# lzzcd001/MeshDiffusion

Measured on NVIDIA H100. Metric: denoising sample-steps/sec at res-64 (4x64^3), uncond_gen PC sampler, higher is better.
Workload: dtype bf16x3

## Files before the change

### include/meshdiff_b200.h

```cpp
#ifndef MESHDIFF_B200_H
#define MESHDIFF_B200_H

#ifdef __cplusplus
extern "C" {
#endif

const char* mdb_last_error(void);
int mdb_version(void);

typedef struct mdb_unet mdb_unet;

typedef struct mdb_unet_config {
  int image_size;
  int nf;
  int n_levels;
  int ch_mult[8];
  int num_res_blocks;
  int level0_blocks;
  int n_attn;
  int attn_resolutions[4];
  int num_channels;
  int stem_ksize;
  int use_pos_bias;
  int max_batch;
  int precision;
  int training;
} mdb_unet_config;

int mdb_unet_create(const mdb_unet_config* cfg, mdb_unet** out);
int mdb_unet_create_dry(const mdb_unet_config* cfg, mdb_unet** out);
void mdb_unet_destroy(mdb_unet* net);

int mdb_unet_num_params(mdb_unet* net);
int mdb_unet_param_info(mdb_unet* net, int idx, const char** name, long long* numel, int* ndim, long long* shape8);
int mdb_unet_set_param(mdb_unet* net, const char* name, const float* src, long long numel, int src_is_device,
                       void* stream);
int mdb_unet_set_params(mdb_unet* net, int count, const char* const* names, const float* const* srcs, const long long* numels,
                        void* stream);
int mdb_unet_get_param(mdb_unet* net, const char* name, float* dst, long long numel, int dst_is_device, void* stream);
int mdb_unet_commit(mdb_unet* net, void* stream);
int mdb_unet_forward(mdb_unet* net, const float* x, const float* labels, float* out, int batch, void* stream);
int mdb_unet_info(mdb_unet* net, double* flops_per_sample, long long* arena_bytes, int* n_gemm_launches, int* n_steps);
int mdb_unet_gemm_ops(mdb_unet* net, int i, const char** name, double* flops, double* fill_bytes);
int mdb_unet_gemm_slots(mdb_unet* net, int i, int* a_slots, int* b_slots, int* smem_bytes);
int mdb_unet_gemm_tiles(mdb_unet* net, int i, int* work_items, int* splits, int* ksteps, int* entry_ksteps, int* block_n);
int mdb_unet_profile(mdb_unet* net, const float* x, const float* labels, float* out, int batch, void* stream,
                     char* names_buf, int names_len, float* ms, int max_steps, int* n_steps);

int mdb_unet_set_dropout(mdb_unet* net, float p, unsigned long long seed);
int mdb_unet_backward(mdb_unet* net, const float* dout, float* grads, long long grads_numel, int batch, int accumulate,
                      void* stream);
int mdb_unet_grad_offset(mdb_unet* net, const char* name, long long* offset);
int mdb_unet_backward_input(mdb_unet* net, const float* dout, float* dx, float* grads, long long grads_numel, int batch,
                            int accumulate, void* stream);
int mdb_unet_grad_ready(mdb_unet* net, const char* name, int* n_launches);
int mdb_unet_backward_marked(mdb_unet* net, const float* dout, float* grads, long long grads_numel, int batch,
                             int accumulate, const int* mark_steps, void* const* mark_events, int n_marks, void* stream);
int mdb_unet_debug_stats(mdb_unet* net, long long* host_out, long long capacity, long long* count);
int mdb_unet_train_info(mdb_unet* net, double* bwd_flops_per_sample, int* n_bwd_steps, long long* total_param_numel);
int mdb_unet_profile_backward(mdb_unet* net, const float* dout, float* grads, int batch, void* stream, char* names_buf,
                              int names_len, float* ms, int max_steps, int* n_steps);

int mdb_fingerprint(const void* const* ptrs_dev, const long long* numels_dev, int n, unsigned long long* out_dev,
                    void* stream);

typedef struct mdb_sampler_cond {
  const float* partial;
  long long partial_bstride;
  const float* partial_mask;
  long long mask_bstride;
  int channel;
  float mean_coef, std;
  const float* noise;
} mdb_sampler_cond;

int mdb_sampler_update(const float* eps, float* x, float* x_mean, const float* noise, const float* mask, float beta,
                       float std, long long voxels, int channels, int batch, unsigned long long seed,
                       unsigned long long offset, const mdb_sampler_cond* cond , void* stream);
int mdb_sampler_run(mdb_unet* net, float* x, float* x_mean, const float* mask, const float* labels,
                    const float* betas, const float* stds, int n_steps, int batch, unsigned long long seed,
                    float* eps_buf, float* labels_buf, int step0, const mdb_sampler_cond* cond ,
                    const float* cond_mean_coefs, const float* cond_stds, int cond_until, void* stream);

typedef struct mdb_solver_step {
  float label;
  float sigma, inv_alpha;
  float c_x, c_0, c_1, c_z;
  float cond_coef, cond_std;
} mdb_solver_step;

int mdb_solver_update(const float* eps, float* x, float* x0_hist, const float* mask, const mdb_solver_step* step,
                      long long voxels, int channels, int batch, const float* noise ,
                      unsigned long long seed, unsigned long long offset, const mdb_sampler_cond* cond ,
                      void* stream);
int mdb_solver_run(mdb_unet* net, float* x, float* x0_hist, const float* mask, const mdb_solver_step* steps, int n_steps,
                   int batch, unsigned long long seed, float* eps_buf, float* labels_buf, int step0,
                   const mdb_sampler_cond* cond , int cond_until, void* stream);

typedef struct mdb_repaint_entry {
  int kind;
  float label;
  float sigma, inv_alpha;
  float c_x, c_0, c_1, c_z;
  float known_coef, known_std;
} mdb_repaint_entry;

typedef struct mdb_repaint_known {
  const float* known;
  long long known_bstride;
  const float* mask;
  long long mask_bstride;
  unsigned channels;
  const float* noise;
} mdb_repaint_known;

int mdb_repaint_update(const float* eps, float* x, float* x0_hist, const float* mask, const mdb_repaint_entry* entry,
                       long long voxels, int channels, int batch, const float* noise ,
                       unsigned long long seed, unsigned long long offset, const mdb_repaint_known* known ,
                       void* stream);
int mdb_repaint_run(mdb_unet* net, float* x, float* x0_hist, const float* mask, const mdb_repaint_entry* entries,
                    int n_entries, int batch, unsigned long long seed, float* eps_buf, float* labels_buf, int step0,
                    const mdb_repaint_known* known , void* stream);

int mdb_ddpm_loss(const float* pred, const float* noise, const float* mask, double mask_sum, float* loss_out,
                  float* grad_pred, double* scratch, int batch, int channels, long long voxels, void* stream);
int mdb_ddpm_perturb(const float* x0, const float* noise, const float* mask, const float* sqrt_ac,
                     const float* sqrt_1mac, float* out, int batch, int channels, long long voxels, void* stream);
int mdb_chunk_elems(void);
int mdb_grad_clip_coef(const float* const* grads_dev, const long long* numels_dev, const int* chunks_dev, int n_chunks,
                       float max_norm, float* coef_out, float* total_norm_out, double* scratch, void* stream);
int mdb_adam_ema_step(float* const* params_dev, const float* const* grads_dev, float* const* exp_avg_dev,
                      float* const* exp_avg_sq_dev, float* const* ema_dev, const long long* numels_dev,
                      const int* chunks_dev, int n_chunks, float lr, float beta1, float beta2, float eps,
                      float weight_decay, int step, const float* clip_coef_dev, float ema_decay, void* stream);
int mdb_ema_update(float* const* ema_dev, const float* const* params_dev, const long long* numels_dev,
                   const int* chunks_dev, int n_chunks, float ema_decay, void* stream);

int mdb_allreduce_grads(void* nccl_comm, float* grads, long long numel, int world_size, void* stream);

int mdb_conv3d(const void* x, int batch, int cin, int z, int y_, int x_, const float* w, const float* bias, int cout,
               int ksize, int stride, void* out, const float* rowbias, const void* residual, long long* stats,
               int precision, void* stream);
int mdb_groupnorm_act(const void* x, const long long* stats, const float* gamma, const float* beta, void* y, int batch,
                      long long voxels, int channels, int silu, int precision, void* stream);

int mdb_conv3d_backward(const void* dy, const void* x, const float* w, int batch, int cin, int cout, int z, int y_,
                        int x_, int ksize, int stride, float* dw, void* dx, void* stream);
int mdb_conv3d_backward_prec(const void* dy, const void* x, const float* w, int batch, int cin, int cout, int z, int y_,
                             int x_, int ksize, int stride, float* dw, void* dx, int precision, void* stream);
int mdb_groupnorm_act_backward(const void* x, const long long* stats, const float* gamma, const float* beta,
                               void* da, const void* add, void* dx, float* dgamma, float* dbeta, int batch,
                               long long voxels, int channels, int silu, float dropout_p, unsigned long long seed,
                               void* stream);
int mdb_groupnorm_act_backward_prec(const void* x, const long long* stats, const float* gamma, const float* beta,
                                    void* da, const void* add, void* dx, float* dgamma, float* dbeta, int batch,
                                    long long voxels, int channels, int silu, float dropout_p, unsigned long long seed,
                                    int precision, void* stream);

int mdb_marching_tets_prepare(const int* tets_host, int n_tets, int n_verts, int max_batch, void** handle);
void mdb_marching_tets_destroy(void* handle);
int mdb_marching_tets_info(void* handle, int* n_edges, int* uv_grid_n);
int mdb_marching_tets_uvs(void* handle, float* uvs, void* stream);
int mdb_marching_tets_count(void* handle, const float* sdf, int batch, int* counts_host, void* stream);
int mdb_marching_tets_extract(void* handle, const float* pos, long long pos_batch_stride, const float* sdf, int batch,
                              float* verts, long long* faces, long long* uv_idx, long long* face_to_tet,
                              long long* valid_vert_idx, const long long* vert_off, const long long* face_off,
                              const long long* vv_off, void* stream);
int mdb_marching_tets_vertex_ids(void* handle, int batch, unsigned* out, void* stream);
int mdb_marching_tets_backward(void* handle, const float* pos, long long pos_batch_stride, const float* sdf, int batch,
                               const unsigned* vertex_ids, const float* grad_verts, const long long* vert_off,
                               float* grad_pos, float* grad_sdf, void* stream);

int mdb_mesh_auto_normals(const float* v_pos, const long long* faces, int n_verts, int n_faces, float* v_nrm, float* f_nrm,
                          long long* scratch, void* stream);
int mdb_mesh_compute_tangents(const float* v_pos, const long long* t_pos_idx, const float* v_tex, const long long* t_tex_idx,
                              const float* v_nrm, const long long* t_nrm_idx, int n_nrm, int n_faces, float* v_tng,
                              long long* scratch, void* stream);

int mdb_mesh_sample_points(const float* verts, const long long* faces, const long long* vert_off, const long long* face_off,
                           int n_meshes, int n_points, const float* uniforms, unsigned long long seed, long long first_id,
                           double* cdf, float* points, int* n_written, void* stream);
int mdb_chamfer_matrix(const float* A, int nA, int N, const float* B, int nB, int M, double* out, void* stream);
int mdb_chamfer_pairs(const float* clouds, int n_clouds, int N, const int* pairs, int P, double* cd, double* mean_ab,
                      float* max_ab, void* stream);
int mdb_emd_matrix(const float* A, int nA, const float* B, int nB, int N, float eps, double* out, double* gap, void* stream);
int mdb_lfd_descriptors(const int* face_id, int n_images, int res, const float* ray_cs, const double* dft,
                        unsigned char* desc, int* n_inside, void* stream);
int mdb_lfd_matrix(const unsigned char* A, int nA, const unsigned char* B, int nB, const signed char* perms, int* out,
                   void* stream);

int mdb_pflow_drift_div(const float* x, const float* e, const float* h, const float* g, const float* mask, float beta, float std,
                        float* drift, double* div, int batch, int channels, long long voxels, void* stream);

int mdb_raster_depth(const float* verts, const long long* faces, const long long* vert_off, const long long* face_off,
                     const int* job_mesh, const float* mvp, int n_jobs, int res, unsigned long long* scratch, float* depth,
                     int* face_id, int* n_behind, void* stream);
int mdb_visible_tets(const float* pos, long long pos_stride, const int* tets, int n_tets, const long long* face_to_tet,
                     const long long* face_off, const int* job_mesh, const float* mvp, int n_jobs, int res, const float* depth,
                     const int* face_id, unsigned char* visible, unsigned char* rast, void* stream);
int mdb_render_shade(const float* verts, const float* v_nrm, const long long* faces, const long long* vert_off,
                     const long long* face_off, const int* job_mesh, const float* mvp, const float* campos, int n_jobs, int res,
                     int ssaa, const int* face_id, const float* sh_coef, const float* kd, const float* bg,
                     const float* srgb_thresholds, unsigned char* rgb, void* stream);

int mdb_carve_vertices(const float* pts, int n_pts, const float* mvp, int n_views, int n_meshes, int res, int window,
                       const float* depth, const int* face_id, unsigned char* outside, void* stream);
int mdb_closest_points(const float* queries, const long long* query_off, int n_meshes, long long max_queries, const float* verts,
                       const long long* faces, const long long* vert_off, const long long* face_off, float* dist2,
                       long long* face, float* closest, void* stream);
int mdb_nearest_vertex(const float* queries, const long long* query_off, int n_meshes, long long max_queries, const float* points,
                       const long long* point_off, float* dist2, long long* index, void* stream);
int mdb_segment_sum(const float* src, int width, const long long* perm, const long long* row_off, long long n_rows, float* out,
                    void* stream);

int mdb_depth_unproject(const float* depth, int n_obs, int res, const float* proj, const float* inv_mv, float max_jump,
                        float* zbuf, int* valid, float* points, unsigned char* edge, void* stream);
int mdb_depth_closest_points(const float* queries, const long long* query_off, int n_obs, long long max_queries, int res,
                             const float* mvp, const float* proj, float radius, const float* points, const int* valid,
                             const unsigned char* edge, float* dist2, float* closest, unsigned char* found, void* stream);

int mdb_slerp_chunks(void);
int mdb_slerp_frames(const float* za, const float* zb, long long n, int pairs, const double* alphas, int frames,
                     double* partial, double* sums, float* coef, float* out, void* stream);

#ifdef __cplusplus
}
#endif
#endif
```

### meshdiffusion_b200/_native.py

```python
import ctypes
import os

_HERE = os.path.dirname(os.path.abspath(__file__))
LIB_PATH = os.path.join(_HERE, "lib", "libmeshdiff_b200.so")

_lib = None


class NativeError(RuntimeError):
    pass


class UNetConfigC(ctypes.Structure):
    _fields_ = [
        ("image_size", ctypes.c_int),
        ("nf", ctypes.c_int),
        ("n_levels", ctypes.c_int),
        ("ch_mult", ctypes.c_int * 8),
        ("num_res_blocks", ctypes.c_int),
        ("level0_blocks", ctypes.c_int),
        ("n_attn", ctypes.c_int),
        ("attn_resolutions", ctypes.c_int * 4),
        ("num_channels", ctypes.c_int),
        ("stem_ksize", ctypes.c_int),
        ("use_pos_bias", ctypes.c_int),
        ("max_batch", ctypes.c_int),
        ("precision", ctypes.c_int),
        ("training", ctypes.c_int),
    ]


class SamplerCondC(ctypes.Structure):
    _fields_ = [
        ("partial", ctypes.c_void_p), ("partial_bstride", ctypes.c_longlong),
        ("partial_mask", ctypes.c_void_p), ("mask_bstride", ctypes.c_longlong),
        ("channel", ctypes.c_int), ("mean_coef", ctypes.c_float), ("std", ctypes.c_float),
        ("noise", ctypes.c_void_p),
    ]


class SolverStepC(ctypes.Structure):
    _fields_ = [(name, ctypes.c_float) for name in
                ("label", "sigma", "inv_alpha", "c_x", "c_0", "c_1", "c_z", "cond_coef", "cond_std")]


class RepaintEntryC(ctypes.Structure):
    _fields_ = [("kind", ctypes.c_int)] + [(name, ctypes.c_float) for name in
                                           ("label", "sigma", "inv_alpha", "c_x", "c_0", "c_1", "c_z", "known_coef",
                                            "known_std")]


class RepaintKnownC(ctypes.Structure):
    _fields_ = [
        ("known", ctypes.c_void_p), ("known_bstride", ctypes.c_longlong),
        ("mask", ctypes.c_void_p), ("mask_bstride", ctypes.c_longlong),
        ("channels", ctypes.c_uint), ("noise", ctypes.c_void_p),
    ]


_vp, _i, _ll, _f, _u64, _d = ctypes.c_void_p, ctypes.c_int, ctypes.c_longlong, ctypes.c_float, ctypes.c_ulonglong, ctypes.c_double
SIGNATURES = {
    "mdb_last_error": (ctypes.c_char_p, []),
    "mdb_version": (_i, []),
    "mdb_unet_create": (_i, [ctypes.POINTER(UNetConfigC), ctypes.POINTER(_vp)]),
    "mdb_unet_create_dry": (_i, [ctypes.POINTER(UNetConfigC), ctypes.POINTER(_vp)]),
    "mdb_unet_destroy": (None, [_vp]),
    "mdb_unet_num_params": (_i, [_vp]),
    "mdb_unet_param_info": (_i, [_vp, _i, ctypes.POINTER(ctypes.c_char_p), ctypes.POINTER(_ll), ctypes.POINTER(_i), ctypes.POINTER(_ll)]),
    "mdb_unet_set_param": (_i, [_vp, ctypes.c_char_p, _vp, _ll, _i, _vp]),
    "mdb_unet_get_param": (_i, [_vp, ctypes.c_char_p, _vp, _ll, _i, _vp]),
    "mdb_unet_commit": (_i, [_vp, _vp]),
    "mdb_unet_set_params": (_i, [_vp, _i, _vp, _vp, _vp, _vp]),
    "mdb_unet_forward": (_i, [_vp, _vp, _vp, _vp, _i, _vp]),
    "mdb_unet_info": (_i, [_vp, ctypes.POINTER(_d), ctypes.POINTER(_ll), ctypes.POINTER(_i), ctypes.POINTER(_i)]),
    "mdb_unet_gemm_ops": (_i, [_vp, _i, ctypes.POINTER(ctypes.c_char_p), ctypes.POINTER(_d), ctypes.POINTER(_d)]),
    "mdb_unet_gemm_slots": (_i, [_vp, _i, ctypes.POINTER(_i), ctypes.POINTER(_i), ctypes.POINTER(_i)]),
    "mdb_unet_gemm_tiles": (_i, [_vp, _i, ctypes.POINTER(_i), ctypes.POINTER(_i), ctypes.POINTER(_i), ctypes.POINTER(_i),
                                 ctypes.POINTER(_i)]),
    "mdb_unet_profile": (_i, [_vp, _vp, _vp, _vp, _i, _vp, ctypes.c_char_p, _i, ctypes.POINTER(_f), _i, ctypes.POINTER(_i)]),
    "mdb_unet_set_dropout": (_i, [_vp, _f, _u64]),
    "mdb_unet_backward": (_i, [_vp, _vp, _vp, _ll, _i, _i, _vp]),
    "mdb_unet_grad_offset": (_i, [_vp, ctypes.c_char_p, ctypes.POINTER(_ll)]),
    "mdb_unet_backward_input": (_i, [_vp, _vp, _vp, _vp, _ll, _i, _i, _vp]),
    "mdb_unet_grad_ready": (_i, [_vp, ctypes.c_char_p, ctypes.POINTER(_i)]),
    "mdb_unet_backward_marked": (_i, [_vp, _vp, _vp, _ll, _i, _i, ctypes.POINTER(_i), ctypes.POINTER(_vp), _i, _vp]),
    "mdb_unet_debug_stats": (_i, [_vp, _vp, _ll, ctypes.POINTER(_ll)]),
    "mdb_unet_train_info": (_i, [_vp, ctypes.POINTER(_d), ctypes.POINTER(_i), ctypes.POINTER(_ll)]),
    "mdb_unet_profile_backward": (_i, [_vp, _vp, _vp, _i, _vp, ctypes.c_char_p, _i, ctypes.POINTER(_f), _i, ctypes.POINTER(_i)]),
    "mdb_fingerprint": (_i, [_vp, _vp, _i, _vp, _vp]),
    "mdb_sampler_update": (_i, [_vp, _vp, _vp, _vp, _vp, _f, _f, _ll, _i, _i, _u64, _u64, ctypes.POINTER(SamplerCondC), _vp]),
    "mdb_sampler_run": (_i, [_vp, _vp, _vp, _vp, ctypes.POINTER(_f), ctypes.POINTER(_f), ctypes.POINTER(_f), _i, _i, _u64, _vp, _vp,
                             _i, ctypes.POINTER(SamplerCondC), ctypes.POINTER(_f), ctypes.POINTER(_f), _i, _vp]),
    "mdb_solver_update": (_i, [_vp, _vp, _vp, _vp, ctypes.POINTER(SolverStepC), _ll, _i, _i, _vp, _u64, _u64,
                               ctypes.POINTER(SamplerCondC), _vp]),
    "mdb_solver_run": (_i, [_vp, _vp, _vp, _vp, ctypes.POINTER(SolverStepC), _i, _i, _u64, _vp, _vp, _i,
                            ctypes.POINTER(SamplerCondC), _i, _vp]),
    "mdb_repaint_update": (_i, [_vp, _vp, _vp, _vp, ctypes.POINTER(RepaintEntryC), _ll, _i, _i, _vp, _u64, _u64,
                                ctypes.POINTER(RepaintKnownC), _vp]),
    "mdb_repaint_run": (_i, [_vp, _vp, _vp, _vp, ctypes.POINTER(RepaintEntryC), _i, _i, _u64, _vp, _vp, _i,
                             ctypes.POINTER(RepaintKnownC), _vp]),
    "mdb_ddpm_loss": (_i, [_vp, _vp, _vp, _d, _vp, _vp, _vp, _i, _i, _ll, _vp]),
    "mdb_ddpm_perturb": (_i, [_vp, _vp, _vp, _vp, _vp, _vp, _i, _i, _ll, _vp]),
    "mdb_chunk_elems": (_i, []),
    "mdb_grad_clip_coef": (_i, [_vp, _vp, _vp, _i, _f, _vp, _vp, _vp, _vp]),
    "mdb_adam_ema_step": (_i, [_vp, _vp, _vp, _vp, _vp, _vp, _vp, _i, _f, _f, _f, _f, _f, _i, _vp, _f, _vp]),
    "mdb_ema_update": (_i, [_vp, _vp, _vp, _vp, _i, _f, _vp]),
    "mdb_allreduce_grads": (_i, [_vp, _vp, _ll, _i, _vp]),
    "mdb_conv3d": (_i, [_vp, _i, _i, _i, _i, _i, _vp, _vp, _i, _i, _i, _vp, _vp, _vp, _vp, _i, _vp]),
    "mdb_groupnorm_act": (_i, [_vp, _vp, _vp, _vp, _vp, _i, _ll, _i, _i, _i, _vp]),
    "mdb_conv3d_backward": (_i, [_vp, _vp, _vp, _i, _i, _i, _i, _i, _i, _i, _i, _vp, _vp, _vp]),
    "mdb_groupnorm_act_backward": (_i, [_vp, _vp, _vp, _vp, _vp, _vp, _vp, _vp, _vp, _i, _ll, _i, _i, _f, _u64, _vp]),
    "mdb_conv3d_backward_prec": (_i, [_vp, _vp, _vp, _i, _i, _i, _i, _i, _i, _i, _i, _vp, _vp, _i, _vp]),
    "mdb_groupnorm_act_backward_prec": (_i, [_vp, _vp, _vp, _vp, _vp, _vp, _vp, _vp, _vp, _i, _ll, _i, _i, _f, _u64, _i, _vp]),
    "mdb_marching_tets_prepare": (_i, [_vp, _i, _i, _i, ctypes.POINTER(_vp)]),
    "mdb_marching_tets_destroy": (None, [_vp]),
    "mdb_marching_tets_info": (_i, [_vp, ctypes.POINTER(_i), ctypes.POINTER(_i)]),
    "mdb_marching_tets_uvs": (_i, [_vp, _vp, _vp]),
    "mdb_marching_tets_count": (_i, [_vp, _vp, _i, ctypes.POINTER(_i), _vp]),
    "mdb_mesh_auto_normals": (_i, [_vp, _vp, _i, _i, _vp, _vp, _vp, _vp]),
    "mdb_mesh_compute_tangents": (_i, [_vp, _vp, _vp, _vp, _vp, _vp, _i, _i, _vp, _vp, _vp]),
    "mdb_marching_tets_extract": (_i, [_vp, _vp, _ll, _vp, _i, _vp, _vp, _vp, _vp, _vp, _vp, _vp, _vp, _vp]),
    "mdb_marching_tets_vertex_ids": (_i, [_vp, _i, _vp, _vp]),
    "mdb_marching_tets_backward": (_i, [_vp, _vp, _ll, _vp, _i, _vp, _vp, _vp, _vp, _vp, _vp]),
    "mdb_mesh_sample_points": (_i, [_vp, _vp, _vp, _vp, _i, _i, _vp, _u64, _ll, _vp, _vp, _vp, _vp]),
    "mdb_chamfer_matrix": (_i, [_vp, _i, _i, _vp, _i, _i, _vp, _vp]),
    "mdb_chamfer_pairs": (_i, [_vp, _i, _i, _vp, _i, _vp, _vp, _vp, _vp]),
    "mdb_emd_matrix": (_i, [_vp, _i, _vp, _i, _i, _f, _vp, _vp, _vp]),
    "mdb_pflow_drift_div": (_i, [_vp, _vp, _vp, _vp, _vp, _f, _f, _vp, _vp, _i, _i, _ll, _vp]),
    "mdb_raster_depth": (_i, [_vp, _vp, _vp, _vp, _vp, _vp, _i, _i, _vp, _vp, _vp, _vp, _vp]),
    "mdb_visible_tets": (_i, [_vp, _ll, _vp, _i, _vp, _vp, _vp, _vp, _i, _i, _vp, _vp, _vp, _vp, _vp]),
    "mdb_render_shade": (_i, [_vp, _vp, _vp, _vp, _vp, _vp, _vp, _vp, _i, _i, _i, _vp, _vp, _vp, _vp, _vp, _vp, _vp]),
    "mdb_carve_vertices": (_i, [_vp, _i, _vp, _i, _i, _i, _i, _vp, _vp, _vp, _vp]),
    "mdb_closest_points": (_i, [_vp, _vp, _i, _ll, _vp, _vp, _vp, _vp, _vp, _vp, _vp, _vp]),
    "mdb_nearest_vertex": (_i, [_vp, _vp, _i, _ll, _vp, _vp, _vp, _vp, _vp]),
    "mdb_segment_sum": (_i, [_vp, _i, _vp, _vp, _ll, _vp, _vp]),
    "mdb_depth_unproject": (_i, [_vp, _i, _i, _vp, _vp, _f, _vp, _vp, _vp, _vp, _vp]),
    "mdb_depth_closest_points": (_i, [_vp, _vp, _i, _ll, _i, _vp, _vp, _f, _vp, _vp, _vp, _vp, _vp, _vp, _vp]),
    "mdb_lfd_descriptors": (_i, [_vp, _i, _i, _vp, _vp, _vp, _vp, _vp]),
    "mdb_lfd_matrix": (_i, [_vp, _i, _vp, _i, _vp, _vp, _vp]),
    "mdb_slerp_chunks": (_i, []),
    "mdb_slerp_frames": (_i, [_vp, _vp, _ll, _i, ctypes.POINTER(_d), _i, _vp, _vp, _vp, _vp, _vp]),
}


def lib():
    global _lib
    if _lib is not None:
        return _lib
    if not os.path.exists(LIB_PATH):
        from . import build as _build
        _build.build()
    if not os.path.exists(LIB_PATH):
        raise NativeError("libmeshdiff_b200.so is missing and could not be built; there is no fallback path")
    L = ctypes.CDLL(LIB_PATH)
    for name, (res, args) in SIGNATURES.items():
        fn = getattr(L, name)
        fn.restype = res
        fn.argtypes = args
    _lib = L
    return L


def check(code):
    if code != 0:
        raise NativeError(lib().mdb_last_error().decode())


def ptr(t):
    if t is None:
        return None
    return ctypes.c_void_p(t.data_ptr())


def current_stream():
    import torch
    return ctypes.c_void_p(torch.cuda.current_stream().cuda_stream)
```

### meshdiffusion_b200/build.py

```python
import os
import re
import subprocess
import sys

HERE = os.path.dirname(os.path.abspath(__file__))
CSRC = os.path.join(HERE, "csrc")
LIBDIR = os.path.join(HERE, "lib")
LIB = os.path.join(LIBDIR, "libmeshdiff_b200.so")
SOURCES = ["gemm_host.cu", "wgrad_host.cu", "elementwise.cu", "backward.cu", "unet.cu", "unet_train.cu", "marching_tets.cu", "mesh_ops.cu", "train_ops.cu", "pc_metrics.cu", "emd.cu", "likelihood.cu", "raster.cu", "fit.cu", "depth_partial.cu", "interp.cu", "lfd.cu", "repaint.cu", "api.cu"]
ARCH_FLAGS = ["-gencode", "arch=compute_90a,code=sm_90a"]
NVCC_FLAGS = ARCH_FLAGS + [
    "-O3", "-lineinfo", "-std=c++17",
    "-Xcompiler", "-fPIC", "--expt-relaxed-constexpr",
    "-Xptxas", "-v",
]
SERIALISED_WGMMA = ("C7510", "C7520")
NO_STACK_KERNELS = ("gemm_tc_kernel", "wgrad_tc_kernel")
_PROPS = re.compile(r"Function properties for (\S+)")
_FRAME = re.compile(r"(\d+) bytes stack frame, (\d+) bytes spill stores, (\d+) bytes spill loads")


def local_memory_violations(ptxas_report):
    bad, fn = [], None
    for line in ptxas_report.splitlines():
        m = _PROPS.search(line)
        if m:
            fn = m.group(1)
            continue
        m = _FRAME.search(line)
        if m and fn and any(k in fn for k in NO_STACK_KERNELS) and any(int(g) for g in m.groups()):
            bad.append(f"{fn}: {line.strip()}")
        fn = None
    return bad


def _newest_mtime(paths):
    return max(os.path.getmtime(p) for p in paths)


def build(force=False, verbose=False):
    import fcntl
    os.makedirs(LIBDIR, exist_ok=True)
    with open(os.path.join(LIBDIR, ".build.lock"), "w") as lock:
        fcntl.flock(lock, fcntl.LOCK_EX)
        try:
            return _build_locked(force, verbose)
        finally:
            fcntl.flock(lock, fcntl.LOCK_UN)


def _build_locked(force, verbose):
    srcs = [os.path.join(CSRC, s) for s in SOURCES if os.path.exists(os.path.join(CSRC, s))]
    deps = [os.path.join(CSRC, f) for f in os.listdir(CSRC)] + [os.path.join(HERE, "..", "include", "meshdiff_b200.h")]
    if not force and os.path.exists(LIB) and os.path.getmtime(LIB) >= _newest_mtime(deps):
        return LIB
    nvcc = os.environ.get("NVCC", "/usr/local/cuda/bin/nvcc")
    objs = []
    procs = []
    for s in srcs:
        o = os.path.join(LIBDIR, os.path.basename(s)[:-3] + ".o")
        objs.append(o)
        cmd = [nvcc] + NVCC_FLAGS + ["-c", s, "-o", o]
        procs.append((cmd, subprocess.Popen(cmd, stdout=subprocess.PIPE, stderr=subprocess.STDOUT)))
    for cmd, p in procs:
        out, _ = p.communicate()
        out = out.decode()
        if verbose or p.returncode != 0:
            sys.stderr.write(out)
        if p.returncode != 0:
            raise RuntimeError("nvcc failed: " + " ".join(cmd))
        serialised = [line for line in out.splitlines() if any(code in line for code in SERIALISED_WGMMA)]
        if serialised:
            raise RuntimeError("ptxas serialised wgmma in " + cmd[-3] + ":\n" + "\n".join(serialised))
        local = local_memory_violations(out)
        if local:
            raise RuntimeError("local memory in a register-only kernel of " + cmd[-3] + ":\n" + "\n".join(local))
    cmd = [nvcc] + ARCH_FLAGS + ["-shared", "-o", LIB] + objs + ["-lcudart", "-ldl"]
    subprocess.check_call(cmd)
    return LIB


if __name__ == "__main__":
    print(build(force="--force" in sys.argv, verbose="-v" in sys.argv))
```

### meshdiffusion_b200/csrc/act_format.cuh

```cuda
#pragma once
#include <cuda_runtime.h>
#include <cuda_bf16.h>
#include <stdint.h>
#include <cmath>
#include <stdexcept>
#include <string>
#include <type_traits>

namespace mdb {

enum Precision { kBF16 = 0, kTF32 = 1, kBF16X3 = 2 };
constexpr int esize(Precision p) { return p == kTF32 ? 4 : 2; }
constexpr int parts(Precision p) { return p == kBF16X3 ? 2 : 1; }
inline Precision precision_from_int(int v) {
  if (v < 0 || v > 2) throw std::runtime_error("mdb: precision must be 0 (bf16), 1 (tf32) or 2 (bf16x3)");
  return static_cast<Precision>(v);
}

__device__ __forceinline__ float to_tf32_rna(float x) {
  uint32_t u;
  asm("cvt.rna.tf32.f32 %0, %1;" : "=r"(u) : "f"(x));
  return __uint_as_float(u);
}
template <Precision P> using ActElem = std::conditional_t<P == kTF32, float, __nv_bfloat16>;
template <Precision P>
__device__ __forceinline__ float load_split(const ActElem<P>* hi, long long lo_off) {
  if constexpr (P == kTF32) {
    return hi[0];
  } else {
    float x = __bfloat162float(hi[0]);
    if constexpr (P == kBF16X3) x += __bfloat162float(hi[lo_off]);
    return x;
  }
}
template <Precision P>
__device__ __forceinline__ void store_split(ActElem<P>* hi, long long lo_off, float v) {
  if constexpr (P == kTF32) {
    hi[0] = to_tf32_rna(v);
  } else {
    const __nv_bfloat16 hb = __float2bfloat16(v);
    hi[0] = hb;
    if constexpr (P == kBF16X3) hi[lo_off] = __float2bfloat16(v - __bfloat162float(hb));
  }
}

__device__ __forceinline__ void bf16x8_decode(const uint4& raw, float* x) {
  const __nv_bfloat162* h = reinterpret_cast<const __nv_bfloat162*>(&raw);
#pragma unroll
  for (int j = 0; j < 4; ++j) { const float2 f = __bfloat1622float2(h[j]); x[2 * j] = f.x; x[2 * j + 1] = f.y; }
}
__device__ __forceinline__ void bf16x8_decode_add(const uint4& raw, float* x) {
  float l[8];
  bf16x8_decode(raw, l);
#pragma unroll
  for (int j = 0; j < 8; ++j) x[j] += l[j];
}
__device__ __forceinline__ uint4 bf16x8_encode(const float* x) {
  uint4 t;
  __nv_bfloat162* h = reinterpret_cast<__nv_bfloat162*>(&t);
#pragma unroll
  for (int j = 0; j < 4; ++j) h[j] = __floats2bfloat162_rn(x[2 * j], x[2 * j + 1]);
  return t;
}
__device__ __forceinline__ uint4 bf16x8_encode_lo(const uint4& hi, const float* x) {
  const __nv_bfloat162* h = reinterpret_cast<const __nv_bfloat162*>(&hi);
  uint4 t;
  __nv_bfloat162* l = reinterpret_cast<__nv_bfloat162*>(&t);
#pragma unroll
  for (int j = 0; j < 4; ++j) {
    const float2 f = __bfloat1622float2(h[j]);
    l[j] = __floats2bfloat162_rn(x[2 * j] - f.x, x[2 * j + 1] - f.y);
  }
  return t;
}

template <Precision P> constexpr int kVecElems = P == kTF32 ? 4 : 8;
template <Precision P>
__device__ __forceinline__ void decode_vec(const uint4& hi, const uint4& lo, float* x) {
  if constexpr (P == kTF32) {
    x[0] = __uint_as_float(hi.x); x[1] = __uint_as_float(hi.y); x[2] = __uint_as_float(hi.z); x[3] = __uint_as_float(hi.w);
  } else {
    bf16x8_decode(hi, x);
    if constexpr (P == kBF16X3) bf16x8_decode_add(lo, x);
  }
}
template <Precision P>
__device__ __forceinline__ void load_vec(const void* hi, long long lo_bytes, float* x) {
  const uint4 h = __ldg(reinterpret_cast<const uint4*>(hi));
  uint4 l = h;
  if constexpr (P == kBF16X3) l = __ldg(reinterpret_cast<const uint4*>(reinterpret_cast<const char*>(hi) + lo_bytes));
  decode_vec<P>(h, l, x);
}
template <Precision P>
__device__ __forceinline__ void store_vec(void* hi, long long lo_bytes, const float* x) {
  if constexpr (P == kTF32) {
    *reinterpret_cast<float4*>(hi) = make_float4(to_tf32_rna(x[0]), to_tf32_rna(x[1]), to_tf32_rna(x[2]), to_tf32_rna(x[3]));
  } else {
    const uint4 h = bf16x8_encode(x);
    *reinterpret_cast<uint4*>(hi) = h;
    if constexpr (P == kBF16X3) *reinterpret_cast<uint4*>(reinterpret_cast<char*>(hi) + lo_bytes) = bf16x8_encode_lo(h, x);
  }
}

__device__ __forceinline__ unsigned long long drop_hash64(unsigned long long seed, unsigned long long idx) {
  unsigned long long z = idx + seed * 0x9E3779B97F4A7C15ull;
  z = (z ^ (z >> 30)) * 0xBF58476D1CE4E5B9ull;
  z = (z ^ (z >> 27)) * 0x94D049BB133111EBull;
  return z ^ (z >> 31);
}
template <int K>
__device__ __forceinline__ void apply_dropout(float* x, unsigned long long seed, unsigned long long e4, int thresh, float scale) {
  unsigned long long h[K];
#pragma unroll
  for (int i = 0; i < K; ++i) h[i] = drop_hash64(seed, e4 + i);
#pragma unroll
  for (int j = 0; j < 4 * K; ++j) {
    const unsigned r16 = (unsigned)((h[j >> 2] >> (16 * (j & 3))) & 0xFFFFu);
    x[j] = r16 >= (unsigned)thresh ? x[j] * scale : 0.f;
  }
}
struct DropoutParams { int thresh; float scale; };
inline DropoutParams dropout_params(float p) { return {(int)std::lround((double)p * 65536.0), p > 0.f ? 1.f / (1.f - p) : 1.f}; }
inline unsigned long long dropout_layer_seed(unsigned long long seed, int layer) {
  return seed + 0x632BE59BD9B4E019ull * (unsigned long long)(layer + 1);
}

__device__ __forceinline__ float sigmoid_ex2(float x) {
  float e, r;
  asm("ex2.approx.ftz.f32 %0, %1;" : "=f"(e) : "f"(x * -1.4426950408889634f));
  asm("rcp.approx.ftz.f32 %0, %1;" : "=f"(r) : "f"(1.f + e));
  return r;
}
__device__ __forceinline__ float silu_ex2(float x) { return x * sigmoid_ex2(x); }
__device__ __forceinline__ float dsilu_ex2(float y) {
  const float s = sigmoid_ex2(y);
  return s * fmaf(y, 1.f - s, 1.f);
}
__device__ __forceinline__ float dsilu_ex2_half(float h) {
  float e, s;
  asm("ex2.approx.ftz.f32 %0, %1;" : "=f"(e) : "f"(h * -2.8853900817779268f));
  asm("rcp.approx.ftz.f32 %0, %1;" : "=f"(s) : "f"(1.f + e));
  return s * fmaf(2.f * h, 1.f - s, 1.f);
}
__device__ __forceinline__ float silu_tanh(float x) {
  float t;
  asm("tanh.approx.f32 %0, %1;" : "=f"(t) : "f"(0.5f * x));
  const float h = 0.5f * x;
  return fmaf(h, t, h);
}
__device__ __forceinline__ float dsilu_tanh_half(float h) {
  float th;
  asm("tanh.approx.f32 %0, %1;" : "=f"(th) : "f"(h));
  return fmaf(0.5f, h * fmaf(-th, th, 1.f), fmaf(0.5f, th, 0.5f));
}
__device__ __forceinline__ float sigmoid_expf(float x) { return 1.f / (1.f + __expf(-x)); }

#define MDB_LAUNCH_CHECK()                                                                              \
  do {                                                                                                  \
    cudaError_t _e = cudaGetLastError();                                                                \
    if (_e != cudaSuccess) throw std::runtime_error(std::string("mdb launch: ") + cudaGetErrorString(_e)); \
  } while (0)

inline int grid_for(long long work_items, int threads) {
  long long b = (work_items + threads - 1) / threads;
  const long long cap = 132LL * 8;
  if (b > cap) b = cap;
  return b < 1 ? 1 : (int)b;
}

}
```

### meshdiffusion_b200/csrc/api.cu

```cuda
#include "../../include/meshdiff_b200.h"
#include "unet.h"
#include <cstring>
#include <cmath>

using namespace mdb;

static thread_local std::string g_err;
namespace mdb { void set_last_error(const std::string& msg) { g_err = msg; } }

#define MDB_API_BEGIN try {
#define MDB_API_END                         \
  }                                         \
  catch (const std::exception& e) {         \
    g_err = e.what();                       \
    return 1;                               \
  }                                         \
  catch (...) {                             \
    g_err = "mdb: unknown error";           \
    return 2;                               \
  }                                         \
  return 0;

struct mdb_unet { UNet* net; };

extern "C" {

const char* mdb_last_error(void) { return g_err.c_str(); }
int mdb_version(void) { return 100; }

static int create_impl(const mdb_unet_config* c, mdb_unet** out, bool dry) {
  MDB_API_BEGIN
  if (!c || !out) throw std::runtime_error("mdb: null argument");
  UNetConfig u;
  u.image_size = c->image_size; u.nf = c->nf; u.n_levels = c->n_levels;
  for (int i = 0; i < 8; ++i) u.ch_mult[i] = c->ch_mult[i];
  u.num_res_blocks = c->num_res_blocks; u.level0_blocks = c->level0_blocks;
  u.n_attn = c->n_attn;
  for (int i = 0; i < 4; ++i) u.attn_resolutions[i] = c->attn_resolutions[i];
  u.num_channels = c->num_channels; u.stem_ksize = c->stem_ksize; u.use_pos_bias = c->use_pos_bias;
  u.max_batch = c->max_batch; u.precision = c->precision; u.training = c->training;
  auto* h = new mdb_unet;
  h->net = nullptr;
  try { h->net = new UNet(u, dry); } catch (...) { delete h; throw; }
  *out = h;
  MDB_API_END
}

int mdb_unet_create(const mdb_unet_config* c, mdb_unet** out) { return create_impl(c, out, false); }
int mdb_unet_create_dry(const mdb_unet_config* c, mdb_unet** out) { return create_impl(c, out, true); }

void mdb_unet_destroy(mdb_unet* n) {
  if (!n) return;
  delete n->net;
  delete n;
}

int mdb_unet_num_params(mdb_unet* n) { return n ? (int)n->net->params().size() : -1; }

int mdb_unet_param_info(mdb_unet* n, int idx, const char** name, long long* numel, int* ndim, long long* shape8) {
  MDB_API_BEGIN
  const auto& ps = n->net->params();
  if (idx < 0 || idx >= (int)ps.size()) throw std::runtime_error("mdb: parameter index out of range");
  if (name) *name = ps[idx].name.c_str();
  if (numel) *numel = ps[idx].numel;
  if (ndim) *ndim = (int)ps[idx].shape.size();
  if (shape8) for (size_t i = 0; i < ps[idx].shape.size() && i < 8; ++i) shape8[i] = ps[idx].shape[i];
  MDB_API_END
}

int mdb_unet_set_param(mdb_unet* n, const char* name, const float* src, long long numel, int dev, void* stream) {
  MDB_API_BEGIN
  n->net->set_param(name, src, numel, dev != 0, (cudaStream_t)stream);
  MDB_API_END
}

int mdb_unet_set_params(mdb_unet* n, int count, const char* const* names, const float* const* srcs, const long long* numels,
                        void* stream) {
  MDB_API_BEGIN
  for (int i = 0; i < count; ++i) n->net->set_param(names[i], srcs[i], numels[i], true, (cudaStream_t)stream);
  MDB_API_END
}

int mdb_unet_get_param(mdb_unet* n, const char* name, float* dst, long long numel, int dev, void* stream) {
  MDB_API_BEGIN
  n->net->get_param(name, dst, numel, dev != 0, (cudaStream_t)stream);
  MDB_API_END
}

int mdb_unet_commit(mdb_unet* n, void* stream) {
  MDB_API_BEGIN
  n->net->commit((cudaStream_t)stream);
  MDB_API_END
}

int mdb_unet_forward(mdb_unet* n, const float* x, const float* labels, float* out, int B, void* stream) {
  MDB_API_BEGIN
  n->net->forward(x, labels, out, B, (cudaStream_t)stream);
  MDB_API_END
}

int mdb_unet_info(mdb_unet* n, double* flops, long long* arena, int* ngemm, int* nsteps) {
  MDB_API_BEGIN
  if (flops) *flops = n->net->flops_per_sample();
  if (arena) *arena = (long long)n->net->arena_bytes();
  if (ngemm) *ngemm = n->net->num_gemm_launches();
  if (nsteps) *nsteps = n->net->num_steps();
  MDB_API_END
}

int mdb_unet_gemm_ops(mdb_unet* n, int i, const char** name, double* flops, double* fill_bytes) {
  MDB_API_BEGIN
  if (i < 0 || i >= n->net->num_gemm_launches()) throw std::runtime_error("mdb: GEMM launch index out of range");
  const GemmOp& g = n->net->gemm(i);
  if (name) *name = g.name.c_str();
  if (flops) *flops = g.flops;
  if (fill_bytes) *fill_bytes = g.fill_bytes();
  MDB_API_END
}

int mdb_unet_gemm_slots(mdb_unet* n, int i, int* a_slots, int* b_slots, int* smem_bytes) {
  MDB_API_BEGIN
  if (i < 0 || i >= n->net->num_gemm_launches()) throw std::runtime_error("mdb: GEMM launch index out of range");
  int a = 0, b = 0, sm = 0;
  n->net->gemm(i).slots(a, b, sm);
  if (a_slots) *a_slots = a;
  if (b_slots) *b_slots = b;
  if (smem_bytes) *smem_bytes = sm;
  MDB_API_END
}

int mdb_unet_gemm_tiles(mdb_unet* n, int i, int* work_items, int* splits, int* ksteps, int* entry_ksteps, int* block_n) {
  MDB_API_BEGIN
  if (i < 0 || i >= n->net->num_gemm_launches()) throw std::runtime_error("mdb: GEMM launch index out of range");
  const GemmOp& g = n->net->gemm(i);
  const int s = g.p.splits > 1 ? g.p.splits : 1;
  int nk = 0;
  for (const LoadEntry& e : g.loads) nk = e.nk > nk ? e.nk : nk;
  if (work_items) *work_items = g.p.tx * g.p.ty * g.p.tz * g.p.tb * g.p.n_tiles_n * s;
  if (splits) *splits = s;
  if (ksteps) *ksteps = g.ksteps;
  if (entry_ksteps) *entry_ksteps = nk;
  if (block_n) *block_n = g.block_n;
  MDB_API_END
}

int mdb_unet_profile(mdb_unet* n, const float* x, const float* labels, float* out, int B, void* stream, char* names,
                     int names_len, float* ms, int max_steps, int* nsteps) {
  MDB_API_BEGIN
  auto r = n->net->profile(x, labels, out, B, (cudaStream_t)stream);
  std::string all;
  int k = 0;
  for (auto& p : r) {
    if (k >= max_steps) break;
    all += p.first; all += "\n";
    ms[k++] = p.second;
  }
  if ((int)all.size() + 1 > names_len) throw std::runtime_error("mdb: names buffer too small");
  std::memcpy(names, all.c_str(), all.size() + 1);
  if (nsteps) *nsteps = k;
  MDB_API_END
}

int mdb_unet_set_dropout(mdb_unet* n, float p, unsigned long long seed) {
  MDB_API_BEGIN
  n->net->set_dropout(p, seed);
  MDB_API_END
}

int mdb_unet_backward(mdb_unet* n, const float* dout, float* grads, long long grads_numel, int B, int accumulate, void* stream) {
  MDB_API_BEGIN
  if (grads_numel != n->net->total_param_numel()) throw std::runtime_error("mdb: gradient buffer has the wrong size");
  n->net->backward(dout, grads, B, accumulate != 0, (cudaStream_t)stream);
  MDB_API_END
}

int mdb_unet_backward_marked(mdb_unet* n, const float* dout, float* grads, long long grads_numel, int B, int accumulate,
                             const int* mark_steps, void* const* mark_events, int n_marks, void* stream) {
  MDB_API_BEGIN
  if (grads_numel != n->net->total_param_numel()) throw std::runtime_error("mdb: gradient buffer has the wrong size");
  if (n_marks > 0 && (!mark_steps || !mark_events)) throw std::runtime_error("mdb: null mark arrays");
  n->net->backward(dout, grads, B, accumulate != 0, (cudaStream_t)stream, mark_steps, mark_events, n_marks);
  MDB_API_END
}

int mdb_unet_backward_input(mdb_unet* n, const float* dout, float* dx, float* grads, long long grads_numel, int B, int accumulate,
                            void* stream) {
  MDB_API_BEGIN
  if (grads && grads_numel != n->net->total_param_numel()) throw std::runtime_error("mdb: gradient buffer has the wrong size");
  n->net->backward_input(dout, dx, grads, B, accumulate != 0, (cudaStream_t)stream);
  MDB_API_END
}

int mdb_unet_grad_ready(mdb_unet* n, const char* name, int* step) {
  MDB_API_BEGIN
  *step = n->net->grad_ready_step(name);
  MDB_API_END
}

int mdb_unet_grad_offset(mdb_unet* n, const char* name, long long* off) {
  MDB_API_BEGIN
  *off = n->net->grad_offset(name);
  MDB_API_END
}

int mdb_unet_debug_stats(mdb_unet* n, long long* host_out, long long capacity, long long* count) {
  MDB_API_BEGIN
  const long long c = (long long)n->net->stats_count();
  if (count) *count = c;
  if (host_out) {
    if (capacity < c) throw std::runtime_error("mdb: stats buffer too small");
    MDB_CUDA_CHECK(cudaMemcpy(host_out, n->net->stats_ptr(), (size_t)c * sizeof(long long), cudaMemcpyDeviceToHost));
  }
  MDB_API_END
}

int mdb_unet_train_info(mdb_unet* n, double* bwd_flops, int* nsteps, long long* numel) {
  MDB_API_BEGIN
  if (bwd_flops) *bwd_flops = n->net->bwd_flops_per_sample();
  if (nsteps) *nsteps = n->net->num_bwd_steps();
  if (numel) *numel = n->net->total_param_numel();
  MDB_API_END
}

int mdb_unet_profile_backward(mdb_unet* n, const float* dout, float* grads, int B, void* stream, char* names, int names_len,
                              float* ms, int max_steps, int* nsteps) {
  MDB_API_BEGIN
  auto r = n->net->profile_backward(dout, grads, B, (cudaStream_t)stream);
  std::string all;
  int k = 0;
  for (auto& p : r) {
    if (k >= max_steps) break;
    all += p.first; all += "\n";
    ms[k++] = p.second;
  }
  if ((int)all.size() + 1 > names_len) throw std::runtime_error("mdb: names buffer too small");
  std::memcpy(names, all.c_str(), all.size() + 1);
  if (nsteps) *nsteps = k;
  MDB_API_END
}

static void set_cond(SamplerUpdateArgs& a, const mdb_sampler_cond* c, float coef, float stdv) {
  if (!c || !c->partial) return;
  if (!c->partial_mask) throw std::runtime_error("mdb: conditional sampling needs partial_mask");
  if (c->channel < 0 || c->channel >= a.C) throw std::runtime_error("mdb: partial_channel out of range");
  a.cond_partial = c->partial; a.cond_partial_bs = c->partial_bstride;
  a.cond_pmask = c->partial_mask; a.cond_pmask_bs = c->mask_bstride;
  a.cond_channel = c->channel; a.cond_coef = coef; a.cond_std = stdv; a.cond_noise = c->noise;
}

int mdb_sampler_update(const float* eps, float* x, float* x_mean, const float* noise, const float* mask, float beta,
                       float stdv, long long V, int C, int B, unsigned long long seed, unsigned long long offset,
                       const mdb_sampler_cond* cond, void* stream) {
  MDB_API_BEGIN
  SamplerUpdateArgs a{};
  a.eps = eps; a.x = x; a.x_mean = x_mean; a.noise = noise; a.mask = mask; a.beta = beta; a.stdv = stdv;
  a.V = V; a.C = C; a.seed = seed; a.offset = offset;
  if (cond) set_cond(a, cond, cond->mean_coef, cond->std);
  launch_sampler_update(a, B, (cudaStream_t)stream);
  MDB_API_END
}

__global__ void fingerprint_kernel(const unsigned int* const* ptrs, const long long* numels, unsigned long long* out) {
  const int t = blockIdx.y;
  const unsigned int* p = ptrs[t];
  const long long n = numels[t];
  unsigned long long h = 0;
  for (long long i = blockIdx.x * (long long)blockDim.x + threadIdx.x; i < n; i += (long long)gridDim.x * blockDim.x)
    h += (unsigned long long)p[i] * (0x9E3779B97F4A7C15ull * (unsigned long long)(i + 1) | 1ull);
  for (int o = 16; o; o >>= 1) h += __shfl_xor_sync(0xffffffffu, h, o);
  if ((threadIdx.x & 31) == 0 && h) atomicAdd(out + t, h);
}

int mdb_fingerprint(const void* const* ptrs_dev, const long long* numels_dev, int n, unsigned long long* out_dev, void* stream) {
  MDB_API_BEGIN
  cudaStream_t s = (cudaStream_t)stream;
  MDB_CUDA_CHECK(cudaMemsetAsync(out_dev, 0, (size_t)n * 8, s));
  fingerprint_kernel<<<dim3(64, n), 256, 0, s>>>(reinterpret_cast<const unsigned int* const*>(ptrs_dev), numels_dev, out_dev);
  MDB_CUDA_CHECK(cudaGetLastError());
  MDB_API_END
}

__global__ void fill_kernel(float* p, float v, int n) {
  const int i = blockIdx.x * blockDim.x + threadIdx.x;
  if (i < n) p[i] = v;
}

int mdb_sampler_run(mdb_unet* n, float* x, float* x_mean, const float* mask, const float* labels, const float* betas,
                    const float* stds, int n_steps, int B, unsigned long long seed, float* eps_buf, float* labels_buf,
                    int step0, const mdb_sampler_cond* cond, const float* cond_mean_coefs, const float* cond_stds,
                    int cond_until, void* stream) {
  MDB_API_BEGIN
  cudaStream_t s = (cudaStream_t)stream;
  const UNetConfig& c = n->net->cfg();
  const long long V = (long long)c.image_size * c.image_size * c.image_size;
  if (cond && cond->partial && (!cond_mean_coefs || !cond_stds)) throw std::runtime_error("mdb: conditional run needs the marginal_prob tables");
  if (cond && cond->noise) throw std::runtime_error("mdb: mdb_sampler_run draws its noise in-kernel (cond->noise must be NULL)");
  for (int i = 0; i < n_steps; ++i) {
    fill_kernel<<<(B + 127) / 128, 128, 0, s>>>(labels_buf, labels[i], B);
    n->net->forward(x, labels_buf, eps_buf, B, s, true);
    SamplerUpdateArgs a{};
    a.eps = eps_buf; a.x = x; a.x_mean = x_mean; a.noise = nullptr; a.mask = mask; a.beta = betas[i]; a.stdv = stds[i];
    a.V = V; a.C = c.num_channels; a.seed = seed; a.offset = 4ull * (unsigned long long)(step0 + i);
    if (cond && step0 + i < cond_until) set_cond(a, cond, cond_mean_coefs[i], cond_stds[i]);
    launch_sampler_update(a, B, s);
  }
  MDB_API_END
}

static SolverUpdateArgs solver_args(const float* eps, float* x, float* x0_hist, const float* mask, const mdb_solver_step& st,
                                    long long V, int C, const mdb_sampler_cond* c) {
  SolverUpdateArgs a{};
  a.eps = eps; a.x = x; a.x0_hist = x0_hist; a.mask = mask;
  a.sigma = st.sigma; a.inv_alpha = st.inv_alpha; a.c_x = st.c_x; a.c_0 = st.c_0; a.c_1 = st.c_1; a.c_z = st.c_z;
  a.V = V; a.C = C;
  if (c && c->partial) {
    if (!c->partial_mask) throw std::runtime_error("mdb: conditional sampling needs partial_mask");
    if (c->channel < 0 || c->channel >= C) throw std::runtime_error("mdb: partial_channel out of range");
    a.cond_partial = c->partial; a.cond_partial_bs = c->partial_bstride;
    a.cond_pmask = c->partial_mask; a.cond_pmask_bs = c->mask_bstride;
    a.cond_channel = c->channel; a.cond_coef = st.cond_coef; a.cond_std = st.cond_std; a.cond_noise = c->noise;
  }
  return a;
}

int mdb_solver_update(const float* eps, float* x, float* x0_hist, const float* mask, const mdb_solver_step* step,
                      long long V, int C, int B, const float* noise, unsigned long long seed, unsigned long long offset,
                      const mdb_sampler_cond* cond, void* stream) {
  MDB_API_BEGIN
  if (!step) throw std::runtime_error("mdb: mdb_solver_update needs a step");
  if (V <= 0 || C <= 0 || B <= 0) throw std::runtime_error("mdb: mdb_solver_update needs positive voxels, channels, batch");
  SolverUpdateArgs a = solver_args(eps, x, x0_hist, mask, *step, V, C, cond);
  a.noise = noise; a.seed = seed; a.offset = offset;
  launch_solver_update(a, B, (cudaStream_t)stream);
  MDB_API_END
}

int mdb_solver_run(mdb_unet* n, float* x, float* x0_hist, const float* mask, const mdb_solver_step* steps, int n_steps,
                   int B, unsigned long long seed, float* eps_buf, float* labels_buf, int step0,
                   const mdb_sampler_cond* cond, int cond_until, void* stream) {
  MDB_API_BEGIN
  cudaStream_t s = (cudaStream_t)stream;
  const UNetConfig& c = n->net->cfg();
  const long long V = (long long)c.image_size * c.image_size * c.image_size;
  if (n_steps > 0 && !steps) throw std::runtime_error("mdb: mdb_solver_run needs the step table");
  if (cond && cond->noise) throw std::runtime_error("mdb: mdb_solver_run draws its noise in-kernel (cond->noise must be NULL)");
  for (int i = 0; i < n_steps; ++i) {
    fill_kernel<<<(B + 127) / 128, 128, 0, s>>>(labels_buf, steps[i].label, B);
    n->net->forward(x, labels_buf, eps_buf, B, s, true);
    SolverUpdateArgs a = solver_args(eps_buf, x, x0_hist, mask, steps[i], V, c.num_channels,
                                     step0 + i < cond_until ? cond : nullptr);
    a.noise = nullptr; a.seed = seed; a.offset = 4ull * (unsigned long long)(step0 + i);
    launch_solver_update(a, B, s);
  }
  MDB_API_END
}

static RepaintArgs repaint_args(const float* eps, float* x, float* x0_hist, const float* mask, const mdb_repaint_entry& e,
                                long long V, int C, const mdb_repaint_known* k) {
  if (e.kind != 0 && e.kind != 1) throw std::runtime_error("mdb: repaint entry kind must be 0 (denoise) or 1 (renoise)");
  RepaintArgs a{};
  a.renoise = e.kind; a.eps = eps; a.x = x; a.x0_hist = x0_hist; a.mask = mask;
  a.sigma = e.sigma; a.inv_alpha = e.inv_alpha; a.c_x = e.c_x; a.c_0 = e.c_0; a.c_1 = e.c_1; a.c_z = e.c_z;
  a.V = V; a.C = C;
  if (k && k->known && k->channels) {
    if (!k->mask) throw std::runtime_error("mdb: the kept region needs its mask");
    if (C > 32 || (C < 32 && (k->channels >> C) != 0u)) throw std::runtime_error("mdb: repaint channel set outside the channels");
    a.known = k->known; a.known_bs = k->known_bstride; a.kmask = k->mask; a.kmask_bs = k->mask_bstride;
    a.channels = k->channels; a.coef = e.known_coef; a.std = e.known_std; a.known_noise = k->noise;
  }
  return a;
}

int mdb_repaint_update(const float* eps, float* x, float* x0_hist, const float* mask, const mdb_repaint_entry* entry,
                       long long V, int C, int B, const float* noise, unsigned long long seed, unsigned long long offset,
                       const mdb_repaint_known* known, void* stream) {
  MDB_API_BEGIN
  if (!entry) throw std::runtime_error("mdb: mdb_repaint_update needs an entry");
  if (V <= 0 || C <= 0 || B <= 0) throw std::runtime_error("mdb: mdb_repaint_update needs positive voxels, channels, batch");
  RepaintArgs a = repaint_args(eps, x, x0_hist, mask, *entry, V, C, known);
  if (!a.renoise && !eps) throw std::runtime_error("mdb: a denoise entry needs the network output");
  a.noise = noise; a.seed = seed; a.offset = offset;
  launch_repaint_update(a, B, (cudaStream_t)stream);
  MDB_API_END
}

int mdb_repaint_run(mdb_unet* n, float* x, float* x0_hist, const float* mask, const mdb_repaint_entry* entries,
                    int n_entries, int B, unsigned long long seed, float* eps_buf, float* labels_buf, int step0,
                    const mdb_repaint_known* known, void* stream) {
  MDB_API_BEGIN
  cudaStream_t s = (cudaStream_t)stream;
  const UNetConfig& c = n->net->cfg();
  const long long V = (long long)c.image_size * c.image_size * c.image_size;
  if (n_entries > 0 && !entries) throw std::runtime_error("mdb: mdb_repaint_run needs the entry table");
  if (known && known->noise) throw std::runtime_error("mdb: mdb_repaint_run draws its noise in-kernel (known->noise must be NULL)");
  for (int i = 0; i < n_entries; ++i) {
    RepaintArgs a = repaint_args(eps_buf, x, x0_hist, mask, entries[i], V, c.num_channels, known);
    if (!a.renoise) {
      fill_kernel<<<(B + 127) / 128, 128, 0, s>>>(labels_buf, entries[i].label, B);
      n->net->forward(x, labels_buf, eps_buf, B, s, true);
    }
    a.noise = nullptr; a.seed = seed; a.offset = 4ull * (unsigned long long)(step0 + i);
    launch_repaint_update(a, B, s);
  }
  MDB_API_END
}

int mdb_conv3d(const void* x, int B, int cin, int z, int y_, int x_, const float* w, const float* bias, int cout,
               int ksize, int stride, void* out, const float* rowbias, const void* residual, long long* stats,
               int precision, void* stream) {
  MDB_API_BEGIN
  cudaStream_t s = (cudaStream_t)stream;
  const Precision pr = precision_from_int(precision);
  const int xo = x_ / stride, yo = y_ / stride, zo = z / stride;
  GemmOp g;
  g.set_output(pr, xo, yo, zo, B, cout, out, cout, false);
  Act a; a.ptr = const_cast<void*>(x); a.C = cin; a.X = x_; a.Y = y_; a.Z = z; a.B = B;
  if (ksize == 1) g.add_pointwise({a}, w, false);
  else g.add_conv({a}, w, ksize, stride);
  if (bias) g.set_bias(bias);
  if (rowbias) g.set_rowbias(rowbias, cout);
  if (residual) g.set_residual(residual, cout, (long long)xo * yo * zo * cout, false);
  if (stats) g.set_stats(stats);
  g.finalize();
  g.upload(s);
  g.repack(s);
  g.launch(s);
  MDB_CUDA_CHECK(cudaStreamSynchronize(s));
  MDB_API_END
}

int mdb_groupnorm_act(const void* x, const long long* stats, const float* gamma, const float* beta, void* y, int B,
                      long long V, int C, int silu, int precision, void* stream) {
  MDB_API_BEGIN
  if (!stats) throw std::runtime_error("mdb: GroupNorm needs the per-channel statistics of x (stats)");
  cudaStream_t s = (cudaStream_t)stream;
  NormActArgs na{};
  na.x0 = x; na.C0 = C; na.ld0 = C; na.x1 = nullptr; na.C1 = 0; na.ld1 = 0;
  na.y = y; na.voxels = V; na.silu = silu; na.prec = precision_from_int(precision);
  na.stats0 = stats; na.stats1 = nullptr; na.gamma = gamma; na.beta = beta; na.groups = 32; na.eps = 1e-6f;
  launch_norm_act(na, B, s);
  MDB_CUDA_CHECK(cudaStreamSynchronize(s));
  MDB_API_END
}

int mdb_conv3d_backward(const void* dy, const void* x, const float* w, int B, int cin, int cout, int z, int y_, int x_,
                        int ksize, int stride, float* dw, void* dx, void* stream) {
  return mdb_conv3d_backward_prec(dy, x, w, B, cin, cout, z, y_, x_, ksize, stride, dw, dx, 0, stream);
}

int mdb_conv3d_backward_prec(const void* dy, const void* x, const float* w, int B, int cin, int cout, int z, int y_, int x_,
                             int ksize, int stride, float* dw, void* dx, int precision, void* stream) {
  MDB_API_BEGIN
  cudaStream_t s = (cudaStream_t)stream;
  const Precision pr = precision_from_int(precision);
  if (pr == kTF32) throw std::runtime_error("mdb: conv3d backward takes bf16 (0) or bf16x3 (2) operands");
  const int xo = x_ / stride, yo = y_ / stride, zo = z / stride;
  Act ady; ady.ptr = const_cast<void*>(dy); ady.C = cout; ady.X = xo; ady.Y = yo; ady.Z = zo; ady.B = B;
  Act ax; ax.ptr = const_cast<void*>(x); ax.C = cin; ax.X = x_; ax.Y = y_; ax.Z = z; ax.B = B;
  if (dw) {
    const int T = ksize * ksize * ksize;
    const WgradPlan pl = plan_wgrad(xo, yo, zo, B, cout, cin, ksize, stride, pr);
    float* scratch = nullptr;
    MDB_CUDA_CHECK(cudaMalloc(&scratch, pl.scratch_bytes));
    WgradOut o; o.ptr = dw; o.sm = (long long)cin * T; o.sn = T; o.st = 1;
    WgradOp op;
    op.init(ady, ax, ksize, stride, o, scratch, pr);
    op.launch(s, B, false);
    MDB_CUDA_CHECK(cudaStreamSynchronize(s));
    cudaFree(scratch);
  }
  if (dx) {
    if (stride != 1) throw std::runtime_error("mdb: conv3d data gradient entry point supports stride 1");
    GemmOp g;
    g.set_output(pr, x_, y_, z, B, cin, dx, cin, false);
    if (ksize == 1) { WSrc ws{w, 1, (long long)cin, 0, cout}; g.add_pointwise_w({ady}, &ws); }
    else g.add_conv_dgrad(ady, w, cin, ksize);
    g.finalize();
    g.upload(s);
    g.repack(s);
    g.launch(s);
    MDB_CUDA_CHECK(cudaStreamSynchronize(s));
  }
  MDB_API_END
}

int mdb_groupnorm_act_backward(const void* x, const long long* stats, const float* gamma, const float* beta, void* da,
                               const void* add, void* dx, float* dgamma, float* dbeta, int B, long long V, int C, int silu,
                               float dropout_p, unsigned long long seed, void* stream) {
  return mdb_groupnorm_act_backward_prec(x, stats, gamma, beta, da, add, dx, dgamma, dbeta, B, V, C, silu, dropout_p, seed, 0, stream);
}

int mdb_groupnorm_act_backward_prec(const void* x, const long long* stats, const float* gamma, const float* beta, void* da,
                                    const void* add, void* dx, float* dgamma, float* dbeta, int B, long long V, int C, int silu,
                                    float dropout_p, unsigned long long seed, int precision, void* stream) {
  MDB_API_BEGIN
  if (!stats) throw std::runtime_error("mdb: GroupNorm backward needs the forward statistics of x (stats)");
  cudaStream_t s = (cudaStream_t)stream;
  const Precision pr = precision_from_int(precision);
  if (pr == kTF32) throw std::runtime_error("mdb: GroupNorm backward takes bf16 (0) or bf16x3 (2) operands");
  float *part = nullptr, *sums = nullptr;
  MDB_CUDA_CHECK(cudaMalloc(&part, (size_t)kBwdPartRows(B) * C * 2 * sizeof(float)));
  MDB_CUDA_CHECK(cudaMalloc(&sums, (size_t)B * C * 2 * sizeof(float)));
  GnBwdArgs a{};
  a.x0 = x; a.C0 = C; a.ld0 = C; a.stats0 = stats; a.gamma = gamma; a.beta = beta; a.da = da;
  a.voxels = V; a.silu = silu; a.groups = 32; a.eps = 1e-6f;
  const DropoutParams d = dropout_params(dropout_p);
  a.drop_thresh = d.thresh; a.drop_scale = d.scale; a.seed = seed;
  a.part = part; a.sums = sums; a.dgamma = dgamma; a.dbeta = dbeta; a.accumulate = 0;
  a.dx = dx; a.add0 = add; a.add0_ld = C;
  a.prec = pr;
  launch_gn_bwd_reduce(a, B, s);
  launch_gn_bwd_apply(a, B, s);
  MDB_CUDA_CHECK(cudaStreamSynchronize(s));
  cudaFree(part); cudaFree(sums);
  MDB_API_END
}

}
```

### meshdiffusion_b200/csrc/ptx.cuh

```cuda
#pragma once
#include <cuda.h>
#include <cuda_runtime.h>
#include <cuda_bf16.h>
#include <stdint.h>
#include <stdio.h>

namespace mdb {

__device__ __forceinline__ uint32_t smem_u32(const void* p) {
  return static_cast<uint32_t>(__cvta_generic_to_shared(p));
}

__device__ __forceinline__ void mbar_init(uint32_t bar, uint32_t count) {
  asm volatile("mbarrier.init.shared::cta.b64 [%0], %1;" ::"r"(bar), "r"(count) : "memory");
}
__device__ __forceinline__ void fence_barrier_init() {
  asm volatile("fence.mbarrier_init.release.cluster;" ::: "memory");
}
__device__ __forceinline__ void fence_proxy_async() {
  asm volatile("fence.proxy.async.shared::cta;" ::: "memory");
}
__device__ __forceinline__ void mbar_expect_tx(uint32_t bar, uint32_t bytes) {
  asm volatile("mbarrier.arrive.expect_tx.shared::cta.b64 _, [%0], %1;" ::"r"(bar), "r"(bytes) : "memory");
}
__device__ __forceinline__ void mbar_arrive(uint32_t bar) {
  asm volatile("mbarrier.arrive.shared::cta.b64 _, [%0];" ::"r"(bar) : "memory");
}
__device__ __forceinline__ void mbar_wait(uint32_t bar, uint32_t parity) {
  asm volatile(
      "{\n\t.reg .pred p;\n\t.reg .u32 n;\n\tmov.u32 n, 0;\n"
      "MDB_WAIT:\n\t"
      "mbarrier.try_wait.parity.shared::cta.b64 p, [%0], %1;\n\t"
      "@p bra MDB_DONE;\n\t"
      "add.u32 n, n, 1;\n\t"
      "setp.lt.u32 p, n, 16777216;\n\t"
      "@p bra MDB_WAIT;\n\t"
      "trap;\n"
      "MDB_DONE:\n\t}"
      :: "r"(bar), "r"(parity) : "memory");
}

__device__ __forceinline__ void tma_prefetch_desc(const void* desc) {
  asm volatile("prefetch.tensormap [%0];" ::"l"(reinterpret_cast<uint64_t>(desc)) : "memory");
}
__device__ __forceinline__ void tma_load_5d(const void* desc, uint32_t bar, uint32_t dst, int c0, int c1, int c2,
                                            int c3, int c4) {
  asm volatile(
      "cp.async.bulk.tensor.5d.shared::cluster.global.mbarrier::complete_tx::bytes"
      " [%0], [%1, {%3, %4, %5, %6, %7}], [%2];"
      :
      : "r"(dst), "l"(reinterpret_cast<uint64_t>(desc)), "r"(bar), "r"(c0), "r"(c1), "r"(c2), "r"(c3), "r"(c4)
      : "memory");
}
__device__ __forceinline__ void tma_load_3d(const void* desc, uint32_t bar, uint32_t dst, int c0, int c1, int c2) {
  asm volatile(
      "cp.async.bulk.tensor.3d.shared::cluster.global.mbarrier::complete_tx::bytes"
      " [%0], [%1, {%3, %4, %5}], [%2];"
      :
      : "r"(dst), "l"(reinterpret_cast<uint64_t>(desc)), "r"(bar), "r"(c0), "r"(c1), "r"(c2)
      : "memory");
}
__device__ __forceinline__ void tma_store_5d(const void* desc, uint32_t src, int c0, int c1, int c2, int c3, int c4) {
  asm volatile(
      "cp.async.bulk.tensor.5d.global.shared::cta.bulk_group [%0, {%2, %3, %4, %5, %6}], [%1];"
      :
      : "l"(reinterpret_cast<uint64_t>(desc)), "r"(src), "r"(c0), "r"(c1), "r"(c2), "r"(c3), "r"(c4)
      : "memory");
}
__device__ __forceinline__ void bulk_commit() { asm volatile("cp.async.bulk.commit_group;" ::: "memory"); }
template <int N>
__device__ __forceinline__ void bulk_wait_read() { asm volatile("cp.async.bulk.wait_group.read %0;" ::"n"(N) : "memory"); }
template <int N>
__device__ __forceinline__ void bulk_wait() { asm volatile("cp.async.bulk.wait_group %0;" ::"n"(N) : "memory"); }
__device__ __forceinline__ unsigned long long globaltimer() {
  unsigned long long t;
  asm volatile("mov.u64 %0, %%globaltimer;" : "=l"(t));
  return t;
}

__device__ __forceinline__ uint64_t make_wgmma_desc(uint32_t saddr, uint32_t lbo_bytes, uint32_t sbo_bytes) {
  return static_cast<uint64_t>((saddr & 0x3FFFFu) >> 4) | (static_cast<uint64_t>((lbo_bytes >> 4) & 0x3FFFu) << 16) |
         (static_cast<uint64_t>((sbo_bytes >> 4) & 0x3FFFu) << 32) | (static_cast<uint64_t>(1) << 62);
}
__device__ __forceinline__ void wgmma_fence() { asm volatile("wgmma.fence.sync.aligned;" ::: "memory"); }
__device__ __forceinline__ void wgmma_commit() { asm volatile("wgmma.commit_group.sync.aligned;" ::: "memory"); }
template <int N>
__device__ __forceinline__ void wgmma_wait() { asm volatile("wgmma.wait_group.sync.aligned %0;" ::"n"(N) : "memory"); }
template <int N>
__device__ __forceinline__ void fence_operands(float (&d)[N]) {
#pragma unroll
  for (int i = 0; i < N; ++i) asm volatile("" : "+f"(d[i])::"memory");
}

template <int TA, int TB>
__device__ __forceinline__ void wgmma_m64n32k16_bf16(float (&d)[16], uint64_t a, uint64_t b, uint32_t scale_d) {
  asm volatile(
      "{\n\t.reg .pred p;\n\tsetp.ne.b32 p, %18, 0;\n\t"
      "wgmma.mma_async.sync.aligned.m64n32k16.f32.bf16.bf16 "
      "{%0, %1, %2, %3, %4, %5, %6, %7, %8, %9, %10, %11, %12, %13, %14, %15}, "
      "%16, %17, p, 1, 1, %19, %20;\n\t}"
      : "+f"(d[0]), "+f"(d[1]), "+f"(d[2]), "+f"(d[3]), "+f"(d[4]), "+f"(d[5]), "+f"(d[6]), "+f"(d[7]), "+f"(d[8]), "+f"(d[9]), "+f"(d[10]), "+f"(d[11]), "+f"(d[12]), "+f"(d[13]), "+f"(d[14]), "+f"(d[15])
      : "l"(a), "l"(b), "r"(scale_d), "n"(TA), "n"(TB));
}
__device__ __forceinline__ void wgmma_m64n32k8_tf32(float (&d)[16], uint64_t a, uint64_t b, uint32_t scale_d) {
  asm volatile(
      "{\n\t.reg .pred p;\n\tsetp.ne.b32 p, %18, 0;\n\t"
      "wgmma.mma_async.sync.aligned.m64n32k8.f32.tf32.tf32 "
      "{%0, %1, %2, %3, %4, %5, %6, %7, %8, %9, %10, %11, %12, %13, %14, %15}, "
      "%16, %17, p, 1, 1;\n\t}"
      : "+f"(d[0]), "+f"(d[1]), "+f"(d[2]), "+f"(d[3]), "+f"(d[4]), "+f"(d[5]), "+f"(d[6]), "+f"(d[7]), "+f"(d[8]), "+f"(d[9]), "+f"(d[10]), "+f"(d[11]), "+f"(d[12]), "+f"(d[13]), "+f"(d[14]), "+f"(d[15])
      : "l"(a), "l"(b), "r"(scale_d));
}
template <int TA, int TB>
__device__ __forceinline__ void wgmma_m64n128k16_bf16(float (&d)[64], uint64_t a, uint64_t b, uint32_t scale_d) {
  asm volatile(
      "{\n\t.reg .pred p;\n\tsetp.ne.b32 p, %66, 0;\n\t"
      "wgmma.mma_async.sync.aligned.m64n128k16.f32.bf16.bf16 "
      "{%0, %1, %2, %3, %4, %5, %6, %7, %8, %9, %10, %11, %12, %13, %14, %15, %16, %17, %18, %19, %20, %21, %22, %23, %24, %25, %26, %27, %28, %29, %30, %31, %32, %33, %34, %35, %36, %37, %38, %39, %40, %41, %42, %43, %44, %45, %46, %47, %48, %49, %50, %51, %52, %53, %54, %55, %56, %57, %58, %59, %60, %61, %62, %63}, "
      "%64, %65, p, 1, 1, %67, %68;\n\t}"
      : "+f"(d[0]), "+f"(d[1]), "+f"(d[2]), "+f"(d[3]), "+f"(d[4]), "+f"(d[5]), "+f"(d[6]), "+f"(d[7]), "+f"(d[8]), "+f"(d[9]), "+f"(d[10]), "+f"(d[11]), "+f"(d[12]), "+f"(d[13]), "+f"(d[14]), "+f"(d[15]), "+f"(d[16]), "+f"(d[17]), "+f"(d[18]), "+f"(d[19]), "+f"(d[20]), "+f"(d[21]), "+f"(d[22]), "+f"(d[23]), "+f"(d[24]), "+f"(d[25]), "+f"(d[26]), "+f"(d[27]), "+f"(d[28]), "+f"(d[29]), "+f"(d[30]), "+f"(d[31]), "+f"(d[32]), "+f"(d[33]), "+f"(d[34]), "+f"(d[35]), "+f"(d[36]), "+f"(d[37]), "+f"(d[38]), "+f"(d[39]), "+f"(d[40]), "+f"(d[41]), "+f"(d[42]), "+f"(d[43]), "+f"(d[44]), "+f"(d[45]), "+f"(d[46]), "+f"(d[47]), "+f"(d[48]), "+f"(d[49]), "+f"(d[50]), "+f"(d[51]), "+f"(d[52]), "+f"(d[53]), "+f"(d[54]), "+f"(d[55]), "+f"(d[56]), "+f"(d[57]), "+f"(d[58]), "+f"(d[59]), "+f"(d[60]), "+f"(d[61]), "+f"(d[62]), "+f"(d[63])
      : "l"(a), "l"(b), "r"(scale_d), "n"(TA), "n"(TB));
}
__device__ __forceinline__ void wgmma_m64n128k8_tf32(float (&d)[64], uint64_t a, uint64_t b, uint32_t scale_d) {
  asm volatile(
      "{\n\t.reg .pred p;\n\tsetp.ne.b32 p, %66, 0;\n\t"
      "wgmma.mma_async.sync.aligned.m64n128k8.f32.tf32.tf32 "
      "{%0, %1, %2, %3, %4, %5, %6, %7, %8, %9, %10, %11, %12, %13, %14, %15, %16, %17, %18, %19, %20, %21, %22, %23, %24, %25, %26, %27, %28, %29, %30, %31, %32, %33, %34, %35, %36, %37, %38, %39, %40, %41, %42, %43, %44, %45, %46, %47, %48, %49, %50, %51, %52, %53, %54, %55, %56, %57, %58, %59, %60, %61, %62, %63}, "
      "%64, %65, p, 1, 1;\n\t}"
      : "+f"(d[0]), "+f"(d[1]), "+f"(d[2]), "+f"(d[3]), "+f"(d[4]), "+f"(d[5]), "+f"(d[6]), "+f"(d[7]), "+f"(d[8]), "+f"(d[9]), "+f"(d[10]), "+f"(d[11]), "+f"(d[12]), "+f"(d[13]), "+f"(d[14]), "+f"(d[15]), "+f"(d[16]), "+f"(d[17]), "+f"(d[18]), "+f"(d[19]), "+f"(d[20]), "+f"(d[21]), "+f"(d[22]), "+f"(d[23]), "+f"(d[24]), "+f"(d[25]), "+f"(d[26]), "+f"(d[27]), "+f"(d[28]), "+f"(d[29]), "+f"(d[30]), "+f"(d[31]), "+f"(d[32]), "+f"(d[33]), "+f"(d[34]), "+f"(d[35]), "+f"(d[36]), "+f"(d[37]), "+f"(d[38]), "+f"(d[39]), "+f"(d[40]), "+f"(d[41]), "+f"(d[42]), "+f"(d[43]), "+f"(d[44]), "+f"(d[45]), "+f"(d[46]), "+f"(d[47]), "+f"(d[48]), "+f"(d[49]), "+f"(d[50]), "+f"(d[51]), "+f"(d[52]), "+f"(d[53]), "+f"(d[54]), "+f"(d[55]), "+f"(d[56]), "+f"(d[57]), "+f"(d[58]), "+f"(d[59]), "+f"(d[60]), "+f"(d[61]), "+f"(d[62]), "+f"(d[63])
      : "l"(a), "l"(b), "r"(scale_d));
}

template <int TA, int TB>
__device__ __forceinline__ void wgmma_m64n64k16_bf16(float (&d)[32], uint64_t a, uint64_t b, uint32_t scale_d) {
  asm volatile(
      "{\n\t.reg .pred p;\n\tsetp.ne.b32 p, %34, 0;\n\t"
      "wgmma.mma_async.sync.aligned.m64n64k16.f32.bf16.bf16 "
      "{%0, %1, %2, %3, %4, %5, %6, %7, %8, %9, %10, %11, %12, %13, %14, %15, %16, %17, %18, %19, %20, %21, %22, %23, %24, %25, %26, %27, %28, %29, %30, %31}, "
      "%32, %33, p, 1, 1, %35, %36;\n\t}"
      : "+f"(d[0]), "+f"(d[1]), "+f"(d[2]), "+f"(d[3]), "+f"(d[4]), "+f"(d[5]), "+f"(d[6]), "+f"(d[7]), "+f"(d[8]), "+f"(d[9]), "+f"(d[10]), "+f"(d[11]), "+f"(d[12]), "+f"(d[13]), "+f"(d[14]), "+f"(d[15]), "+f"(d[16]), "+f"(d[17]), "+f"(d[18]), "+f"(d[19]), "+f"(d[20]), "+f"(d[21]), "+f"(d[22]), "+f"(d[23]), "+f"(d[24]), "+f"(d[25]), "+f"(d[26]), "+f"(d[27]), "+f"(d[28]), "+f"(d[29]), "+f"(d[30]), "+f"(d[31])
      : "l"(a), "l"(b), "r"(scale_d), "n"(TA), "n"(TB));
}
template <int TA, int TB>
__device__ __forceinline__ void wgmma_m64n256k16_bf16(float (&d)[128], uint64_t a, uint64_t b, uint32_t scale_d) {
  asm volatile(
      "{\n\t.reg .pred p;\n\tsetp.ne.b32 p, %130, 0;\n\t"
      "wgmma.mma_async.sync.aligned.m64n256k16.f32.bf16.bf16 "
      "{%0, %1, %2, %3, %4, %5, %6, %7, %8, %9, %10, %11, %12, %13, %14, %15, %16, %17, %18, %19, %20, %21, %22, %23, %24, %25, %26, %27, %28, %29, %30, %31, %32, %33, %34, %35, %36, %37, %38, %39, %40, %41, %42, %43, %44, %45, %46, %47, %48, %49, %50, %51, %52, %53, %54, %55, %56, %57, %58, %59, %60, %61, %62, %63, %64, %65, %66, %67, %68, %69, %70, %71, %72, %73, %74, %75, %76, %77, %78, %79, %80, %81, %82, %83, %84, %85, %86, %87, %88, %89, %90, %91, %92, %93, %94, %95, %96, %97, %98, %99, %100, %101, %102, %103, %104, %105, %106, %107, %108, %109, %110, %111, %112, %113, %114, %115, %116, %117, %118, %119, %120, %121, %122, %123, %124, %125, %126, %127}, "
      "%128, %129, p, 1, 1, %131, %132;\n\t}"
      : "+f"(d[0]), "+f"(d[1]), "+f"(d[2]), "+f"(d[3]), "+f"(d[4]), "+f"(d[5]), "+f"(d[6]), "+f"(d[7]), "+f"(d[8]), "+f"(d[9]), "+f"(d[10]), "+f"(d[11]), "+f"(d[12]), "+f"(d[13]), "+f"(d[14]), "+f"(d[15]), "+f"(d[16]), "+f"(d[17]), "+f"(d[18]), "+f"(d[19]), "+f"(d[20]), "+f"(d[21]), "+f"(d[22]), "+f"(d[23]), "+f"(d[24]), "+f"(d[25]), "+f"(d[26]), "+f"(d[27]), "+f"(d[28]), "+f"(d[29]), "+f"(d[30]), "+f"(d[31]), "+f"(d[32]), "+f"(d[33]), "+f"(d[34]), "+f"(d[35]), "+f"(d[36]), "+f"(d[37]), "+f"(d[38]), "+f"(d[39]), "+f"(d[40]), "+f"(d[41]), "+f"(d[42]), "+f"(d[43]), "+f"(d[44]), "+f"(d[45]), "+f"(d[46]), "+f"(d[47]), "+f"(d[48]), "+f"(d[49]), "+f"(d[50]), "+f"(d[51]), "+f"(d[52]), "+f"(d[53]), "+f"(d[54]), "+f"(d[55]), "+f"(d[56]), "+f"(d[57]), "+f"(d[58]), "+f"(d[59]), "+f"(d[60]), "+f"(d[61]), "+f"(d[62]), "+f"(d[63]), "+f"(d[64]), "+f"(d[65]), "+f"(d[66]), "+f"(d[67]), "+f"(d[68]), "+f"(d[69]), "+f"(d[70]), "+f"(d[71]), "+f"(d[72]), "+f"(d[73]), "+f"(d[74]), "+f"(d[75]), "+f"(d[76]), "+f"(d[77]), "+f"(d[78]), "+f"(d[79]), "+f"(d[80]), "+f"(d[81]), "+f"(d[82]), "+f"(d[83]), "+f"(d[84]), "+f"(d[85]), "+f"(d[86]), "+f"(d[87]), "+f"(d[88]), "+f"(d[89]), "+f"(d[90]), "+f"(d[91]), "+f"(d[92]), "+f"(d[93]), "+f"(d[94]), "+f"(d[95]), "+f"(d[96]), "+f"(d[97]), "+f"(d[98]), "+f"(d[99]), "+f"(d[100]), "+f"(d[101]), "+f"(d[102]), "+f"(d[103]), "+f"(d[104]), "+f"(d[105]), "+f"(d[106]), "+f"(d[107]), "+f"(d[108]), "+f"(d[109]), "+f"(d[110]), "+f"(d[111]), "+f"(d[112]), "+f"(d[113]), "+f"(d[114]), "+f"(d[115]), "+f"(d[116]), "+f"(d[117]), "+f"(d[118]), "+f"(d[119]), "+f"(d[120]), "+f"(d[121]), "+f"(d[122]), "+f"(d[123]), "+f"(d[124]), "+f"(d[125]), "+f"(d[126]), "+f"(d[127])
      : "l"(a), "l"(b), "r"(scale_d), "n"(TA), "n"(TB));
}

template <int N, bool TF32>
__device__ __forceinline__ void wgmma_kmajor(float (&d)[N / 2], uint64_t a, uint64_t b, uint32_t scale_d) {
  if constexpr (N == 256) {
    static_assert(!TF32, "m64n256 is used by the split-bf16 products only");
    wgmma_m64n256k16_bf16<0, 0>(d, a, b, scale_d);
  } else if constexpr (N == 128) {
    if constexpr (TF32) wgmma_m64n128k8_tf32(d, a, b, scale_d); else wgmma_m64n128k16_bf16<0, 0>(d, a, b, scale_d);
  } else if constexpr (N == 64) {
    static_assert(!TF32, "m64n64 is used by the split-bf16 products only");
    wgmma_m64n64k16_bf16<0, 0>(d, a, b, scale_d);
  } else {
    static_assert(N == 32, "wgmma_kmajor is instantiated for N = 32, 64, 128 and 256");
    if constexpr (TF32) wgmma_m64n32k8_tf32(d, a, b, scale_d); else wgmma_m64n32k16_bf16<0, 0>(d, a, b, scale_d);
  }
}

__device__ __forceinline__ bool elect_one() {
  uint32_t pred = 0;
  asm volatile(
      "{\n\t.reg .pred p;\n\t"
      "elect.sync _|p, 0xffffffff;\n\t"
      "selp.u32 %0, 1, 0, p;\n\t}"
      : "=r"(pred));
  return pred != 0;
}

template <int N>
__device__ __forceinline__ void setmaxnreg_inc() { asm volatile("setmaxnreg.inc.sync.aligned.u32 %0;" ::"n"(N)); }
template <int N>
__device__ __forceinline__ void setmaxnreg_dec() { asm volatile("setmaxnreg.dec.sync.aligned.u32 %0;" ::"n"(N)); }

__device__ __forceinline__ void named_bar_sync(int id, int nthreads) {
  asm volatile("bar.sync %0, %1;" ::"r"(id), "r"(nthreads) : "memory");
}

}
```

### meshdiffusion_b200/csrc/unet.cu

```cuda
#include "unet.h"
#include <algorithm>
#include <cmath>

namespace mdb {

size_t Arena::alloc(size_t bytes) {
  bytes = (bytes + 1023) & ~size_t(1023);
  for (size_t i = 0; i < blocks_.size(); ++i) {
    if (blocks_[i].free && blocks_[i].size >= bytes) {
      const size_t off = blocks_[i].off;
      if (blocks_[i].size > bytes) {
        Block rest{off + bytes, blocks_[i].size - bytes, true};
        blocks_[i].size = bytes;
        blocks_.insert(blocks_.begin() + i + 1, rest);
      }
      blocks_[i].free = false;
      return off;
    }
  }
  if (!blocks_.empty() && blocks_.back().free) {
    blocks_.back().size = bytes;
    blocks_.back().free = false;
    end_ = blocks_.back().off + bytes;
    peak_ = std::max(peak_, end_);
    return blocks_.back().off;
  }
  blocks_.push_back({end_, bytes, false});
  end_ += bytes;
  peak_ = std::max(peak_, end_);
  return blocks_.back().off;
}

void Arena::release(size_t off) {
  for (size_t i = 0; i < blocks_.size(); ++i) {
    if (blocks_[i].off == off && !blocks_[i].free) {
      blocks_[i].free = true;
      if (i + 1 < blocks_.size() && blocks_[i + 1].free) {
        blocks_[i].size += blocks_[i + 1].size;
        blocks_.erase(blocks_.begin() + i + 1);
      }
      if (i > 0 && blocks_[i - 1].free) {
        blocks_[i - 1].size += blocks_[i].size;
        blocks_.erase(blocks_.begin() + i);
      }
      if (!blocks_.empty() && blocks_.back().free) {
        end_ = blocks_.back().off;
        blocks_.pop_back();
      }
      return;
    }
  }
  throw std::runtime_error("mdb: arena release of unknown block");
}

void* UNet::dmalloc(size_t bytes, bool zero) {
  if (dry_) return nullptr;
  void* p = nullptr;
  MDB_CUDA_CHECK(cudaMalloc(&p, bytes ? bytes : 16));
  if (zero) MDB_CUDA_CHECK(cudaMemset(p, 0, bytes ? bytes : 16));
  owned_.push_back(p);
  return p;
}

float* UNet::P(const std::string& name, std::vector<long long> shape, bool external, float* slice) {
  auto it = pindex_.find(name);
  if (it == pindex_.end()) {
    ParamInfo pi;
    pi.name = name; pi.shape = shape; pi.numel = 1;
    for (auto d : shape) pi.numel *= d;
    pi.external = external;
    pindex_[name] = (int)params_.size();
    params_.push_back(pi);
    it = pindex_.find(name);
  }
  ParamInfo& pi = params_[it->second];
  if (external) pi.d = slice;
  return pi.d;
}

TensP UNet::new_act(int C, int R, bool stats) {
  auto t = std::make_shared<Tens>();
  t->C = C; t->R = R;
  t->bytes = (size_t)cfg_.max_batch * R * R * R * C * esize(prec_) * parts(prec_);
  t->off = arena_.alloc(t->bytes);
  t->ptr = at(t->off);
  if (stats) {
    const size_t n = (size_t)cfg_.max_batch * C * kStatWords;
    t->stats = dry_ ? nullptr : stats_base_ + stats_cursor_;
    stats_cursor_ += n;
  }
  return t;
}

void UNet::release(TensP& t) {
  if (train_) return;
  arena_.release(t->off);
  t->live = false;
  t.reset();
}

Act UNet::act_of(const TensP& t) const {
  Act a;
  a.ptr = t->ptr; a.C = t->C; a.X = a.Y = a.Z = t->R; a.B = cfg_.max_batch;
  return a;
}

UNet::Scratch UNet::split_begin(int R, int N, int cin_total, int taps) {
  Scratch s;
  s.S = plan_splits(R, R, R, cfg_.max_batch, N, cin_total, taps, prec_);
  if (s.S > 1) {
    const size_t bytes = (size_t)s.S * cfg_.max_batch * R * R * R * N * sizeof(float);
    s.off = arena_.alloc(bytes);
    s.ptr = reinterpret_cast<float*>(at(s.off));
    s.active = true;
  }
  return s;
}
void UNet::split_end(Scratch& s) {
  if (s.active) arena_.release(s.off);
  s.active = false;
}

GemmOp* UNet::new_gemm(const std::string& name, bool commit_time) {
  auto g = std::make_unique<GemmOp>();
  g->name = name;
  GemmOp* raw = g.get();
  if (commit_time) commit_gemms_.push_back(std::move(g));
  else gemms_.push_back(std::move(g));
  return raw;
}

void UNet::gemm_step(std::vector<Step>& steps, GemmOp* g, std::function<void(cudaStream_t, int)> fn, int kind) {
  g->finalize();
  if (!dry_) g->upload(0);
  if (!fn) fn = [g](cudaStream_t s, int B) { g->launch(s, B); };
  steps.push_back({g->name, fn, kind});
}

TensP UNet::gn(const std::string& pname, const std::vector<TensP>& ins, bool silu, int drop_layer) {
  int C = 0;
  for (auto& t : ins) C += t->C;
  const int R = ins[0]->R;
  float* gamma = P(pname + ".weight", {C});
  float* beta = P(pname + ".bias", {C});
  TensP y = new_act(C, R, false);
  NormActArgs na{};
  na.x0 = ins[0]->ptr; na.C0 = ins[0]->C; na.ld0 = ins[0]->C;
  na.x1 = ins.size() > 1 ? ins[1]->ptr : nullptr; na.C1 = ins.size() > 1 ? ins[1]->C : 0; na.ld1 = na.C1;
  na.y = y->ptr; na.voxels = (long long)R * R * R; na.silu = silu ? 1 : 0; na.prec = prec_;
  na.stats0 = ins[0]->stats; na.stats1 = ins.size() > 1 ? ins[1]->stats : nullptr;
  na.gamma = gamma; na.beta = beta; na.groups = 32; na.eps = 1e-6f;
  if (train_ && drop_layer >= 0) {
    add_step("norm_act:" + pname, [na, this, drop_layer](cudaStream_t s, int B) {
      NormActArgs a = na;
      a.drop_thresh = rt_drop_thresh_; a.drop_scale = rt_drop_scale_; a.seed = dropout_layer_seed(rt_seed_, drop_layer);
      launch_norm_act(a, B, s);
    });
  } else {
    add_step("norm_act:" + pname, [na](cudaStream_t s, int B) { launch_norm_act(na, B, s); });
  }
  return y;
}

TensP UNet::resblock(const std::vector<TensP>& ins, int out_ch, int midx) {
  const std::string pre = "all_modules." + std::to_string(midx) + ".";
  int Cin = 0;
  for (auto& t : ins) Cin += t->C;
  const int R = ins[0]->R, mb = cfg_.max_batch;
  const int tdim = 4 * cfg_.nf;

  TensP a = gn(pre + "GroupNorm_0", ins, true);
  float* w0 = P(pre + "Conv_0.weight", {out_ch, Cin, 3, 3, 3});
  float* b0 = P(pre + "Conv_0.bias", {out_ch});
  const int doff = dense_cursor_;
  dense_cursor_ += out_ch;
  P(pre + "Dense_0.weight", {out_ch, tdim}, true, dense_w_ + (size_t)doff * tdim);
  P(pre + "Dense_0.bias", {out_ch}, true, dense_b_ + doff);
  TensP h = new_act(out_ch, R, true);
  Scratch sp0 = split_begin(R, out_ch, Cin, 27);
  GemmOp* g0 = new_gemm("res" + std::to_string(midx) + ".conv0");
  g0->set_output(prec_, R, R, R, mb, out_ch, h->ptr, out_ch, false);
  g0->add_conv({act_of(a)}, w0, 3, 1);
  g0->set_bias(b0);
  g0->set_rowbias(dense_out_ + doff, dense_total_);
  g0->set_stats(h->stats);
  g0->enable_splits(sp0.S, sp0.ptr);
  gemm_step(steps_, g0);
  split_end(sp0);
  release(a);
  TensP a2 = gn(pre + "GroupNorm_1", {h}, true, midx);
  release(h);
  float* w1 = P(pre + "Conv_1.weight", {out_ch, out_ch, 3, 3, 3});
  float* b1 = P(pre + "Conv_1.bias", {out_ch});
  const bool nin = Cin != out_ch;
  float* wn = nullptr; float* bn = nullptr;
  if (nin) {
    wn = P(pre + "NIN_0.W", {Cin, out_ch});
    bn = P(pre + "NIN_0.b", {out_ch});
  } else if (ins.size() != 1) {
    throw std::runtime_error("mdb: identity shortcut over a concatenation is not supported");
  }
  TensP out = new_act(out_ch, R, true);
  Scratch sp1 = split_begin(R, out_ch, out_ch, 27);
  GemmOp* g1 = new_gemm("res" + std::to_string(midx) + ".conv1");
  g1->set_output(prec_, R, R, R, mb, out_ch, out->ptr, out_ch, false);
  g1->add_conv({act_of(a2)}, w1, 3, 1);
  if (nin) {
    std::vector<Act> raw;
    for (auto& t : ins) raw.push_back(act_of(t));
    g1->add_pointwise(raw, wn, true);
    float* bsum = (float*)dmalloc(out_ch * 4);
    commit_steps_.push_back({"bias:" + pre, [=](cudaStream_t s, int) { launch_add_vec(b1, bn, bsum, out_ch, s); }});
    g1->set_bias(bsum);
  } else {
    g1->set_bias(b1);
    g1->set_residual(ins[0]->ptr, out_ch, (long long)R * R * R * out_ch, false);
  }
  g1->set_stats(out->stats);
  g1->enable_splits(sp1.S, sp1.ptr);
  gemm_step(steps_, g1);
  split_end(sp1);
  if (train_) tape_resblock(ins, a, h, a2, out, out_ch, midx, doff);
  release(a2);
  return out;
}

TensP UNet::attn(const TensP& x, int midx) {
  const std::string pre = "all_modules." + std::to_string(midx) + ".";
  const int C = x->C, R = x->R, mb = cfg_.max_batch;
  const int V = R * R * R;
  const int es = esize(prec_);
  TensP hn = gn(pre + "GroupNorm_0", {x}, false);
  float* W[4]; float* Bv[4];
  for (int i = 0; i < 4; ++i) {
    W[i] = P(pre + "NIN_" + std::to_string(i) + ".W", {C, C});
    Bv[i] = P(pre + "NIN_" + std::to_string(i) + ".b", {C});
  }
  TensP qkv = new_act(3 * C, R, false);
  for (int i = 0; i < 3; ++i) {
    GemmOp* g = new_gemm("attn" + std::to_string(midx) + ".nin" + std::to_string(i));
    g->set_output(prec_, R, R, R, mb, C, (char*)qkv->ptr + (size_t)i * C * es, 3 * C, false);
    g->add_pointwise({act_of(hn)}, W[i], true);
    g->set_bias(Bv[i]);
    gemm_step(steps_, g);
  }
  release(hn);
  TensP vT = new_act(C, R, false);
  {
    const void* src = qkv->ptr; void* dst = vT->ptr;
    if (prec_ == kBF16X3) {
      add_step("attn" + std::to_string(midx) + ".vT", [=](cudaStream_t s, int B) {
        launch_transpose_vc(src, 6 * C, 2 * C, dst, B, V, C, es, s, 2 * V);
        launch_transpose_vc(src, 6 * C, 5 * C, (__nv_bfloat16*)dst + V, B, V, C, es, s, 2 * V);
      });
    } else
    add_step("attn" + std::to_string(midx) + ".vT", [=](cudaStream_t s, int B) { launch_transpose_vc(src, 3 * C, 2 * C, dst, B, V, C, es, s); });
  }
  auto S = std::make_shared<Tens>();
  S->bytes = (size_t)mb * V * V * 4;
  S->off = arena_.alloc(S->bytes);
  S->ptr = at(S->off);
  TensP O = new_act(C, R, false);
  GemmOp* gqk = new_gemm("attn" + std::to_string(midx) + ".qk");
  gqk->set_output_strided(prec_, V, 1, 1, mb, V, S->ptr, V, 0, 0, (long long)V * V, true);
  Act q; q.ptr = qkv->ptr; q.C = C; q.ld = 3 * C; q.X = V; q.Y = 1; q.Z = 1; q.B = mb;
  gqk->add_pointwise_w({q}, nullptr);
  gqk->set_b_activation((char*)qkv->ptr + (size_t)C * es, C, V, mb, 3 * C, (long long)V * 3 * C);
  gqk->set_alpha(1.0f / std::sqrt((float)C));
  gemm_step(steps_, gqk);
  float* sp = (float*)S->ptr; const Precision pr = prec_;
  add_step("attn" + std::to_string(midx) + ".softmax", [=](cudaStream_t s, int B) { launch_softmax_rows(sp, (long long)B * V, V, pr, s); });
  GemmOp* gpv = new_gemm("attn" + std::to_string(midx) + ".pv");
  gpv->set_output_strided(prec_, V, 1, 1, mb, C, O->ptr, C, 0, 0, (long long)V * C, false);
  Act pa; pa.ptr = S->ptr; pa.C = V; pa.ld = (prec_ == kBF16) ? 2 * V : V; pa.X = V; pa.Y = 1; pa.Z = 1; pa.B = mb;
  gpv->add_pointwise_w({pa}, nullptr);
  gpv->set_b_activation(vT->ptr, V, C, mb, V, (long long)C * V);
  gemm_step(steps_, gpv);
  if (!train_) arena_.release(S->off);
  { arena_.release(vT->off); vT->live = false; }
  release(qkv);
  TensP out = new_act(C, R, true);
  GemmOp* g3 = new_gemm("attn" + std::to_string(midx) + ".nin3");
  g3->set_output(prec_, R, R, R, mb, C, out->ptr, C, false);
  g3->add_pointwise({act_of(O)}, W[3], true);
  g3->set_bias(Bv[3]);
  g3->set_residual(x->ptr, C, (long long)V * C, false);
  g3->set_stats(out->stats);
  gemm_step(steps_, g3);
  if (train_) tape_attn(x, hn, qkv, S, O, out, midx);
  release(O);
  return out;
}

TensP UNet::downsample(const TensP& x, int midx) {
  const std::string pre = "all_modules." + std::to_string(midx) + ".";
  const int C = x->C, R = x->R / 2;
  float* w = P(pre + "Conv_0.weight", {C, C, 3, 3, 3});
  float* b = P(pre + "Conv_0.bias", {C});
  TensP out = new_act(C, R, true);
  Scratch sp = split_begin(R, C, C, 27);
  GemmOp* g = new_gemm("down" + std::to_string(midx));
  g->set_output(prec_, R, R, R, cfg_.max_batch, C, out->ptr, C, false);
  g->add_conv({act_of(x)}, w, 3, 2);
  g->set_bias(b);
  g->set_stats(out->stats);
  g->enable_splits(sp.S, sp.ptr);
  gemm_step(steps_, g);
  split_end(sp);
  if (train_) tape_downsample(x, out, midx);
  return out;
}

TensP UNet::upsample(const TensP& x, int midx) {
  const std::string pre = "all_modules." + std::to_string(midx) + ".";
  const int C = x->C, R = x->R * 2;
  float* w = P(pre + "Conv_0.weight", {C, C, 3, 3, 3});
  float* b = P(pre + "Conv_0.bias", {C});
  if (!train_) {
    TensP out = new_act(C, R, true);
    const int r = x->R, mb = cfg_.max_batch;
    float* w8 = (float*)dmalloc((size_t)64 * C * C * sizeof(float));
    commit_steps_.push_back({"upw:" + pre, [=](cudaStream_t s, int) { launch_upconv_weights(w, w8, C, C, s); }});
    const long long es = esize(prec_) * parts(prec_);
    for (int par = 0; par < 8; ++par) {
      const int px = par & 1, py = (par >> 1) & 1, pz = par >> 2;
      GemmOp* g = new_gemm("up" + std::to_string(midx) + ".conv.p" + std::to_string(par));
      char* base = (char*)out->ptr + (((long long)pz * R + py) * R + px) * C * es;
      g->set_output_strided(prec_, r, r, r, mb, C, base, 2LL * C, 2LL * R * C, 2LL * R * R * C, (long long)R * R * R * C, false, C);
      g->add_conv_up2(act_of(x), w8 + (size_t)par * C * C * 8, px, py, pz);
      g->set_bias(b);
      g->set_stats(out->stats);
      gemm_step(steps_, g);
    }
    return out;
  }
  TensP up = new_act(C, R, false);
  {
    const void* src = x->ptr; void* dst = up->ptr; const int r = x->R; const int es = esize(prec_);
    const int Cp = C * parts(prec_);
    add_step("up" + std::to_string(midx) + ".nearest", [=](cudaStream_t s, int B) { launch_upsample2x(src, dst, B, r, r, r, Cp, es, s); });
  }
  TensP out = new_act(C, R, true);
  Scratch sp = split_begin(R, C, C, 27);
  GemmOp* g = new_gemm("up" + std::to_string(midx) + ".conv");
  g->set_output(prec_, R, R, R, cfg_.max_batch, C, out->ptr, C, false);
  g->add_conv({act_of(up)}, w, 3, 1);
  g->set_bias(b);
  g->set_stats(out->stats);
  g->enable_splits(sp.S, sp.ptr);
  gemm_step(steps_, g);
  split_end(sp);
  if (train_) tape_upsample(x, up, out, midx);
  release(up);
  return out;
}

void UNet::build() {
  const int nf = cfg_.nf, R0 = cfg_.image_size, mb = cfg_.max_batch, Cin = cfg_.num_channels;
  const int k = cfg_.stem_ksize, T = k * k * k;
  const int KB = kb_elems(prec_);
  const int tdim = 4 * nf;
  arena_.reset();
  stats_cursor_ = 0;
  dense_cursor_ = 0;
  steps_.clear(); commit_steps_.clear(); bwd_steps_.clear();
  gemms_.clear(); commit_gemms_.clear(); bwd_gemms_.clear(); wgrads_.clear();
  grad_ready_.clear();
  auto is_attn = [&](int r) { for (int i = 0; i < cfg_.n_attn; ++i) if (cfg_.attn_resolutions[i] == r) return true; return false; };
  auto blocks_at = [&](int lvl) { return (lvl == 0 && cfg_.level0_blocks > 0) ? cfg_.level0_blocks : cfg_.num_res_blocks; };

  int m = 0;
  float* tw0 = P("all_modules.0.weight", {tdim, nf});
  float* tb0 = P("all_modules.0.bias", {tdim});
  float* tw1 = P("all_modules.1.weight", {tdim, tdim});
  float* tb1 = P("all_modules.1.bias", {tdim});
  m = 2;
  add_step("temb", [=](cudaStream_t s, int B) {
    launch_temb(rt_labels_, tw0, tb0, tw1, tb1, temb_act_, B, nf, s);
    launch_dense(temb_act_, dense_w_, dense_b_, dense_out_, B, tdim, dense_total_, s);
  });
  if (train_) tape_temb();
  float* mask = P("mask", {1, 1, R0, R0, R0});
  if (cfg_.use_pos_bias) P("coords", {1, 3, R0, R0, R0});
  float* posw = P("pos_layer.weight", {nf, 3, k, k, k});
  float* posb = P("pos_layer.bias", {nf});
  float* mw = P("mask_layer.weight", {nf, 1, k, k, k});
  float* mbias = P("mask_layer.bias", {nf});
  (void)posw;
  float* sw = P("all_modules.2.weight", {nf, Cin, k, k, k});
  float* sb = P("all_modules.2.bias", {nf});
  m = 3;
  const int Kpad = ((Cin * T + KB - 1) / KB) * KB;
  const int Kpad_m = ((T + KB - 1) / KB) * KB;
  const long long V0 = (long long)R0 * R0 * R0;
  auto A0 = std::make_shared<Tens>();
  A0->bytes = (size_t)mb * V0 * Kpad * esize(prec_) * parts(prec_);
  A0->off = arena_.alloc(A0->bytes);
  A0->ptr = at(A0->off);
  TensP h0 = new_act(nf, R0, true);
  float* field = (float*)dmalloc(V0 * nf * 4);
  void* Am = dmalloc(V0 * Kpad_m * esize(prec_) * parts(prec_));
  float* fbias = (float*)dmalloc(nf * 4);
  const Precision pr = prec_;
  const bool use_pos = cfg_.use_pos_bias != 0;
  commit_steps_.push_back({"field.bias", [=](cudaStream_t s, int) { launch_add_vec(mbias, use_pos ? posb : nullptr, fbias, nf, s); }});
  commit_steps_.push_back({"field.im2col", [=](cudaStream_t s, int) { launch_im2col(mask, Am, 1, 1, R0, k, Kpad_m, pr, s); }});
  GemmOp* gf = new_gemm("stem.field", true);
  gf->set_output(prec_, R0, R0, R0, 1, nf, field, nf, true);
  Act am; am.ptr = Am; am.C = Kpad_m; am.X = am.Y = am.Z = R0; am.B = 1;
  WSrc wm{mw, (long long)T, 1, 0, T};
  gf->add_pointwise_w({am}, &wm);
  gf->set_bias(fbias);
  gemm_step(commit_steps_, gf, [gf](cudaStream_t s, int) { gf->repack(s); gf->launch(s, 1); });

  void* a0 = A0->ptr;
  add_step("stem.im2col", [=](cudaStream_t s, int B) { launch_im2col(rt_x_, a0, B, Cin, R0, k, Kpad, pr, s); });
  GemmOp* gs = new_gemm("stem.gemm");
  gs->set_output(prec_, R0, R0, R0, mb, nf, h0->ptr, nf, false);
  Act ax; ax.ptr = a0; ax.C = Kpad; ax.X = ax.Y = ax.Z = R0; ax.B = mb;
  WSrc ws{sw, (long long)Cin * T, 1, 0, Cin * T};
  gs->add_pointwise_w({ax}, &ws);
  gs->set_bias(sb);
  gs->set_residual(field, nf, 0, true);
  gs->set_stats(h0->stats);
  gemm_step(steps_, gs);
  arena_.release(A0->off);
  if (train_) tape_stem(h0, Am, Kpad, Kpad_m);

  std::vector<TensP> hs;
  hs.push_back(h0);
  int in_ch = nf;
  for (int lvl = 0; lvl < cfg_.n_levels; ++lvl) {
    const int res = R0 >> lvl;
    for (int b = 0; b < blocks_at(lvl); ++b) {
      const int out_ch = nf * cfg_.ch_mult[lvl];
      TensP h = resblock({hs.back()}, out_ch, m++);
      in_ch = out_ch;
      if (is_attn(res)) {
        TensP h2 = attn(h, m++);
        release(h);
        h = h2;
      }
      hs.push_back(h);
    }
    if (lvl != cfg_.n_levels - 1) hs.push_back(downsample(hs.back(), m++));
  }
  TensP h;
  {
    TensP h1 = resblock({hs.back()}, in_ch, m++);
    TensP h2 = attn(h1, m++);
    release(h1);
    h = resblock({h2}, in_ch, m++);
    release(h2);
  }
  for (int lvl = cfg_.n_levels - 1; lvl >= 0; --lvl) {
    const int res = R0 >> lvl;
    for (int b = 0; b < blocks_at(lvl) + 1; ++b) {
      const int out_ch = nf * cfg_.ch_mult[lvl];
      TensP skip = hs.back();
      hs.pop_back();
      TensP hn = resblock({h, skip}, out_ch, m++);
      release(h);
      release(skip);
      h = hn;
    }
    if (is_attn(res)) {
      TensP h2 = attn(h, m++);
      release(h);
      h = h2;
    }
    if (lvl != 0) {
      TensP u = upsample(h, m++);
      release(h);
      h = u;
    }
  }
  if (!hs.empty()) throw std::runtime_error("mdb: skip stack not empty");
  const std::string head_gn = "all_modules." + std::to_string(m);
  TensP a = gn("all_modules." + std::to_string(m++), {h}, true);
  TensP head_in = h;
  release(h);
  float* hw = P("all_modules." + std::to_string(m) + ".weight", {Cin, nf, k, k, k});
  float* hb = P("all_modules." + std::to_string(m) + ".bias", {Cin});
  ++m;
  if (Cin == 4) {
    const int Np = ((T * Cin + 7) / 8) * 8;
    const bool pf32 = prec_ != kBF16;
    auto Pt = std::make_shared<Tens>();
    Pt->bytes = (size_t)mb * V0 * Np * (pf32 ? 4 : 2);
    Pt->off = arena_.alloc(Pt->bytes);
    Pt->ptr = at(Pt->off);
    GemmOp* g = new_gemm("head.proj");
    g->set_output(prec_, R0, R0, R0, mb, T * Cin, Pt->ptr, Np, pf32);
    WSrc wh{hw, (long long)nf * T, (long long)T, 0, nf, Cin, 1};
    g->add_pointwise_w({act_of(a)}, &wh);
    gemm_step(steps_, g);
    const void* pp = Pt->ptr;
    add_step("head.shift_sum", [=](cudaStream_t s, int B) { launch_tap_shift_sum(pp, Np, pf32 ? 1 : 0, hb, rt_out_, B, R0, k, Cin, s); });
    arena_.release(Pt->off);
  } else {
    GemmOp* g = new_gemm("head.conv");
    g->set_output_strided(prec_, R0, R0, R0, mb, Cin, nullptr, 1, R0, (long long)R0 * R0, (long long)Cin * V0, true);
    g->set_out_col_stride(V0);
    g->add_conv({act_of(a)}, hw, k, 1);
    g->set_bias(hb);
    gemm_step(steps_, g, [g, this](cudaStream_t s, int B) { g->launch(s, B, rt_out_); });
  }
  if (train_) tape_head(head_in, a, head_gn, "all_modules." + std::to_string(m - 1));
  release(a);
  dense_total_ = dense_cursor_;
  long long off = 0;
  for (auto& p : params_) { goff_[p.name] = off; off += p.numel; }
  if (train_) {
    for (auto it = tape_.rbegin(); it != tape_.rend(); ++it) {
      touched_.clear();
      (*it)();
      for (auto& n : touched_) grad_ready_[n] = (int)bwd_steps_.size();
    }
    tape_.clear();
    if (arena_.in_use() != 0) throw std::runtime_error("mdb: training plan leaked " + std::to_string(arena_.in_use()) + " arena bytes");
  }
  flops_ = 0;
  for (auto& g : gemms_) flops_ += g->flops;
  bwd_flops_ = 0;
  for (auto& g : bwd_gemms_) bwd_flops_ += g->flops;
  for (auto& g : wgrads_) bwd_flops_ += g->flops;
}

UNet::UNet(const UNetConfig& cfg, bool dry_only) : cfg_(cfg), prec_(precision_from_int(cfg.precision)) {
  if (cfg_.image_size % (1 << (cfg_.n_levels - 1)) != 0) throw std::runtime_error("mdb: image_size not divisible by 2^(levels-1)");
  if (cfg_.nf % 32 != 0) throw std::runtime_error("mdb: nf must be a multiple of 32 (GroupNorm(32))");
  train_ = cfg_.training != 0;
  if (const char* e = getenv("MDB_GRAPH_MAX_BATCH")) graph_max_batch_ = atoi(e);
  if (train_ && prec_ == kTF32) throw std::runtime_error("mdb: the training plan is built for bf16 or bf16x3 (split bf16) operands");
  dry_ = true;
  build();
  arena_bytes_ = arena_.peak();
  stats_doubles_ = stats_cursor_;
  if (dry_only) return;
  const size_t n_fwd = steps_.size(), n_commit = commit_steps_.size(), n_bwd = bwd_steps_.size();
  dry_ = false;
  arena_base_ = (char*)dmalloc(arena_bytes_, false);
  stats_base_ = (long long*)dmalloc(stats_doubles_ * sizeof(long long));
  const int tdim = 4 * cfg_.nf;
  temb_act_ = (float*)dmalloc((size_t)cfg_.max_batch * tdim * 4);
  dense_w_ = (float*)dmalloc((size_t)dense_total_ * tdim * 4);
  dense_b_ = (float*)dmalloc((size_t)dense_total_ * 4);
  dense_out_ = (float*)dmalloc((size_t)cfg_.max_batch * dense_total_ * 4);
  if (train_) d_dense_out_ = (float*)dmalloc((size_t)cfg_.max_batch * dense_total_ * 4);
  for (auto& p : params_)
    if (!p.external) p.d = (float*)dmalloc(p.numel * 4);
  build();
  if (arena_.peak() != arena_bytes_ || stats_cursor_ != stats_doubles_ || steps_.size() != n_fwd ||
      commit_steps_.size() != n_commit || bwd_steps_.size() != n_bwd)
    throw std::runtime_error("mdb: the plan built over the arena differs from the dry plan that sized it");
  MDB_CUDA_CHECK(cudaDeviceSynchronize());
}

UNet::~UNet() {
  drop_graphs();
  if (capture_stream_) cudaStreamDestroy(capture_stream_);
  gemms_.clear();
  bwd_gemms_.clear();
  wgrads_.clear();
  commit_gemms_.clear();
  for (void* p : owned_) cudaFree(p);
}

void UNet::set_param(const std::string& name, const float* src, long long numel, bool dev, cudaStream_t s) {
  check_runnable();
  auto it = pindex_.find(name);
  if (it == pindex_.end()) throw std::runtime_error("mdb: unknown parameter " + name);
  ParamInfo& p = params_[it->second];
  if (p.numel != numel) throw std::runtime_error("mdb: parameter " + name + " expects " + std::to_string(p.numel) + " elements, got " + std::to_string(numel));
  MDB_CUDA_CHECK(cudaMemcpyAsync(p.d, src, numel * 4, dev ? cudaMemcpyDeviceToDevice : cudaMemcpyHostToDevice, s));
  committed_ = false;
}

void UNet::get_param(const std::string& name, float* dst, long long numel, bool dev, cudaStream_t s) {
  check_runnable();
  auto it = pindex_.find(name);
  if (it == pindex_.end()) throw std::runtime_error("mdb: unknown parameter " + name);
  ParamInfo& p = params_[it->second];
  if (p.numel != numel) throw std::runtime_error("mdb: parameter " + name + " size mismatch");
  MDB_CUDA_CHECK(cudaMemcpyAsync(dst, p.d, numel * 4, dev ? cudaMemcpyDeviceToDevice : cudaMemcpyDeviceToHost, s));
  MDB_CUDA_CHECK(cudaStreamSynchronize(s));
}

void UNet::commit(cudaStream_t s) {
  check_runnable();
  drop_graphs();
  for (auto& st : commit_steps_) st.fn(s, 1);
  for (auto& g : gemms_) g->repack(s);
  for (auto& g : bwd_gemms_) g->repack(s);
  MDB_CUDA_CHECK(cudaStreamSynchronize(s));
  committed_ = true;
}

void UNet::drop_graphs() {
  for (auto& g : graphs_) if (g.exec) cudaGraphExecDestroy(g.exec);
  graphs_.clear();
}

void UNet::forward(const float* x, const float* labels, float* out, int B, cudaStream_t s, bool allow_graph) {
  check_runnable();
  if (!committed_) throw std::runtime_error("mdb: parameters changed, call commit() before forward()");
  if (B < 1 || B > cfg_.max_batch) throw std::runtime_error("mdb: batch out of range");
  rt_x_ = x; rt_labels_ = labels; rt_out_ = out;
  if (allow_graph && !train_ && B <= graph_max_batch_) {
    FwdGraph* fg = nullptr;
    for (auto& g : graphs_) if (g.x == x && g.labels == labels && g.out == out && g.B == B) fg = &g;
    if (!fg) {
      if (graphs_.size() >= 8) drop_graphs();
      graphs_.push_back({x, labels, out, B, 0, nullptr});
      fg = &graphs_.back();
    }
    if (fg->exec) { MDB_CUDA_CHECK(cudaGraphLaunch(fg->exec, s)); return; }
    if (fg->uses++ >= 1) {
      if (!capture_stream_) MDB_CUDA_CHECK(cudaStreamCreateWithFlags(&capture_stream_, cudaStreamNonBlocking));
      cudaGraph_t graph = nullptr;
      MDB_CUDA_CHECK(cudaStreamBeginCapture(capture_stream_, cudaStreamCaptureModeThreadLocal));
      try {
        MDB_CUDA_CHECK(cudaMemsetAsync(stats_base_, 0, stats_doubles_ * sizeof(long long), capture_stream_));
        for (auto& st : steps_) st.fn(capture_stream_, B);
      } catch (...) {
        cudaStreamEndCapture(capture_stream_, &graph);
        if (graph) cudaGraphDestroy(graph);
        throw;
      }
      MDB_CUDA_CHECK(cudaStreamEndCapture(capture_stream_, &graph));
      cudaError_t e = cudaGraphInstantiate(&fg->exec, graph, 0);
      cudaGraphDestroy(graph);
      if (e != cudaSuccess) { fg->exec = nullptr; MDB_CUDA_CHECK(e); }
      MDB_CUDA_CHECK(cudaGraphLaunch(fg->exec, s));
      return;
    }
  }
  MDB_CUDA_CHECK(cudaMemsetAsync(stats_base_, 0, stats_doubles_ * sizeof(long long), s));
  for (auto& st : steps_) st.fn(s, B);
}

std::vector<std::pair<std::string, float>> UNet::profile(const float* x, const float* labels, float* out, int B, cudaStream_t s) {
  check_runnable();
  if (!committed_) throw std::runtime_error("mdb: commit() first");
  rt_x_ = x; rt_labels_ = labels; rt_out_ = out;
  std::vector<std::pair<std::string, float>> res;
  std::vector<cudaEvent_t> ev(steps_.size() + 1);
  for (auto& e : ev) MDB_CUDA_CHECK(cudaEventCreate(&e));
  MDB_CUDA_CHECK(cudaMemsetAsync(stats_base_, 0, stats_doubles_ * sizeof(long long), s));
  MDB_CUDA_CHECK(cudaEventRecord(ev[0], s));
  for (size_t i = 0; i < steps_.size(); ++i) {
    steps_[i].fn(s, B);
    MDB_CUDA_CHECK(cudaEventRecord(ev[i + 1], s));
  }
  MDB_CUDA_CHECK(cudaStreamSynchronize(s));
  for (size_t i = 0; i < steps_.size(); ++i) {
    float ms = 0;
    MDB_CUDA_CHECK(cudaEventElapsedTime(&ms, ev[i], ev[i + 1]));
    res.push_back({steps_[i].name, ms});
  }
  for (auto& e : ev) cudaEventDestroy(e);
  return res;
}

}
```

### meshdiffusion_b200/csrc/unet.h

```cpp
#pragma once
#include <functional>
#include <map>
#include <memory>
#include <string>
#include <vector>
#include "gemm_host.h"
#include "wgrad_host.h"
#include "elementwise.cuh"
#include "backward.cuh"

namespace mdb {

struct UNetConfig {
  int image_size = 64;
  int nf = 128;
  int n_levels = 5;
  int ch_mult[8] = {1, 1, 2, 4, 4, 0, 0, 0};
  int num_res_blocks = 3;
  int level0_blocks = -1;
  int n_attn = 1;
  int attn_resolutions[4] = {16, 0, 0, 0};
  int num_channels = 4;
  int stem_ksize = 3;
  int use_pos_bias = 1;
  int max_batch = 1;
  int precision = 0;
  int training = 0;
};

struct ParamInfo {
  std::string name;
  std::vector<long long> shape;
  long long numel = 0;
  float* d = nullptr;
  bool external = false;
};

class Arena {
 public:
  size_t alloc(size_t bytes);
  void release(size_t off);
  size_t peak() const { return peak_; }
  size_t in_use() const { size_t n = 0; for (auto& b : blocks_) if (!b.free) n += b.size; return n; }
  void reset() { blocks_.clear(); end_ = 0; peak_ = 0; }
 private:
  struct Block { size_t off, size; bool free; };
  std::vector<Block> blocks_;
  size_t end_ = 0, peak_ = 0;
};

struct GradBuf { size_t off = 0; int refs = 0; bool has_cs = false; size_t cs_off = 0; };
struct GradView {
  std::shared_ptr<GradBuf> buf;
  void* ptr = nullptr;
  long long ld = 0;
  int C = 0;
  float* colsum = nullptr;
  long long cs_ld = 0;
  bool valid() const { return buf != nullptr; }
};

struct Tens {
  size_t off = 0, bytes = 0;
  int C = 0, R = 0;
  long long* stats = nullptr;
  void* ptr = nullptr;
  bool live = true;
  GradView grad;
};
typedef std::shared_ptr<Tens> TensP;

class UNet {
 public:
  explicit UNet(const UNetConfig& cfg, bool dry_only = false);
  ~UNet();
  const std::vector<ParamInfo>& params() const { return params_; }
  void set_param(const std::string& name, const float* src, long long numel, bool src_device, cudaStream_t s);
  void get_param(const std::string& name, float* dst, long long numel, bool dst_device, cudaStream_t s);
  void commit(cudaStream_t s);
  void forward(const float* x, const float* labels, float* out, int B, cudaStream_t s, bool allow_graph = false);
  void set_dropout(float p, unsigned long long seed);
  void backward(const float* dout, float* grads, int B, bool accumulate, cudaStream_t s, const int* mark_steps = nullptr,
                void* const* mark_events = nullptr, int n_marks = 0);
  void backward_input(const float* dout, float* dx, float* grads, int B, bool accumulate, cudaStream_t s);
  int grad_ready_step(const std::string& name) const;
  long long grad_offset(const std::string& name) const;
  long long total_param_numel() const;
  int num_bwd_steps() const { return (int)bwd_steps_.size(); }
  size_t stats_count() const { return stats_doubles_; }
  const long long* stats_ptr() const { return stats_base_; }
  double bwd_flops_per_sample() const { return bwd_flops_ / cfg_.max_batch; }
  std::vector<std::pair<std::string, float>> profile_backward(const float* dout, float* grads, int B, cudaStream_t s);
  double flops_per_sample() const { return flops_ / cfg_.max_batch; }
  size_t arena_bytes() const { return arena_bytes_; }
  int num_gemm_launches() const { return (int)gemms_.size(); }
  const GemmOp& gemm(int i) const { return *gemms_.at(i); }
  int num_steps() const { return (int)steps_.size(); }
  const UNetConfig& cfg() const { return cfg_; }
  std::vector<std::pair<std::string, float>> profile(const float* x, const float* labels, float* out, int B, cudaStream_t s);

 private:
  UNetConfig cfg_;
  Precision prec_;
  bool dry_ = true;
  std::vector<ParamInfo> params_;
  std::map<std::string, int> pindex_;
  std::vector<void*> owned_;
  Arena arena_;
  char* arena_base_ = nullptr;
  size_t arena_bytes_ = 0;
  long long* stats_base_ = nullptr;
  size_t stats_doubles_ = 0, stats_cursor_ = 0;
  std::vector<std::unique_ptr<GemmOp>> gemms_;
  std::vector<std::unique_ptr<GemmOp>> commit_gemms_;
  enum StepKind { kAlways = 0, kParamGradOnly = 1, kInputGradOnly = 2 };
  struct Step { std::string name; std::function<void(cudaStream_t, int)> fn; int kind = kAlways; };
  std::vector<Step> steps_, commit_steps_;
  bool committed_ = false;
  double flops_ = 0;
  struct FwdGraph { const float* x; const float* labels; float* out; int B; int uses; cudaGraphExec_t exec; };
  std::vector<FwdGraph> graphs_;
  cudaStream_t capture_stream_ = nullptr;
  int graph_max_batch_ = 8;
  void drop_graphs();
  const float* rt_x_ = nullptr;
  const float* rt_labels_ = nullptr;
  float* rt_out_ = nullptr;
  float* temb_act_ = nullptr;
  float* dense_w_ = nullptr; float* dense_b_ = nullptr; float* dense_out_ = nullptr;
  int dense_total_ = 0, dense_cursor_ = 0;

  void build();
  void check_runnable() const { if (dry_) throw std::runtime_error("mdb: a dry plan cannot run"); }
  float* P(const std::string& name, std::vector<long long> shape, bool external = false, float* slice = nullptr);
  void* dmalloc(size_t bytes, bool zero = true);
  char* at(size_t arena_off) const { return dry_ ? nullptr : arena_base_ + arena_off; }
  TensP new_act(int C, int R, bool stats);
  void release(TensP& t);
  Act act_of(const TensP& t) const;
  GemmOp* new_gemm(const std::string& name, bool commit_time = false);
  void add_step(const std::string& name, std::function<void(cudaStream_t, int)> fn) { steps_.push_back({name, fn}); }
  void gemm_step(std::vector<Step>& steps, GemmOp* g, std::function<void(cudaStream_t, int)> fn = {}, int kind = kAlways);
  struct Scratch { int S = 1; size_t off = 0; float* ptr = nullptr; bool active = false; };
  Scratch split_begin(int R, int N, int cin_total, int taps);
  void split_end(Scratch& s);
  TensP gn(const std::string& pname, const std::vector<TensP>& ins, bool silu, int drop_layer = -1);
  bool train_ = false;
  std::vector<std::function<void()>> tape_;
  std::vector<Step> bwd_steps_;
  std::vector<std::unique_ptr<GemmOp>> bwd_gemms_;
  std::vector<std::unique_ptr<WgradOp>> wgrads_;
  double bwd_flops_ = 0;
  std::map<std::string, long long> goff_;
  mutable std::vector<std::string> touched_;
  std::map<std::string, int> grad_ready_;
  float* rt_grads_ = nullptr; const float* rt_dout_ = nullptr; bool rt_accum_ = false;
  float* rt_dx_ = nullptr;
  bool has_input_grad_ = false;
  int rt_drop_thresh_ = 0; float rt_drop_scale_ = 1.f; unsigned long long rt_seed_ = 0;
  float* d_dense_out_ = nullptr;
  void add_bwd(const std::string& name, std::function<void(cudaStream_t, int)> fn, int kind = kAlways) {
    bwd_steps_.push_back({name, fn, kind});
  }
  void run_backward(const float* dout, float* grads, float* dx, int B, bool accumulate, cudaStream_t s, const int* mark_steps,
                    void* const* mark_events, int n_marks);
  void free_act(const TensP& t);
  GradView new_grad(int C, int R);
  GradView grad_view(const GradView& g, int c0, int C);
  void unref(GradView& g);
  Act act_of_grad(const GradView& g, int R) const;
  long long G(const std::string& name) const;
  struct Tmp { size_t off = 0; void* ptr = nullptr; };
  struct GnFuse {
    std::string pname; std::vector<TensP> ins; bool silu = false; int drop_layer = -1;
    bool on = false; Tmp consts, part; int T = 0, bb = 1;
  };
  void gn_fuse_attach(GnFuse& f, GemmOp* g, int N, int R);
  Tmp tmp_alloc(size_t bytes);
  void tmp_free(Tmp& t);
  GemmOp* new_bwd_gemm(const std::string& name);
  void emit_colsum(const std::string& name, const GradView& t, int R, float* per, long long per_ld, long long g0, long long g1, long long g2);
  void emit_wgrad(const std::string& name, const Act& dy, const Act& x, int ksize, int stride, long long goff, const WgradOut& layout);
  GradView emit_conv_dgrad(const std::string& name, const GradView& dy, int R, const float* w, int cin_total, const GradView* addend, GnFuse* fuse = nullptr);
  GradView emit_pointwise(const std::string& name, const std::vector<Act>& srcs, const std::vector<WSrc>& ws, int N, int R, const GradView* addend, GnFuse* fuse = nullptr);
  GradView emit_gn_backward(const std::string& pname, const std::vector<TensP>& ins, const GradView& da, bool silu, int drop_layer,
                            const GradView* add0, const GradView* add1, GnFuse* fuse = nullptr);
  void tape_resblock(const std::vector<TensP>& ins, TensP a, TensP h, TensP a2, TensP out, int out_ch, int midx, int doff);
  void tape_attn(TensP x, TensP hn, TensP qkv, TensP S, TensP O, TensP out, int midx);
  void tape_downsample(TensP x, TensP out, int midx);
  void tape_upsample(TensP x, TensP up, TensP out, int midx);
  void tape_stem(TensP h0, void* Am, int Kpad, int Kpad_m);
  void tape_head(TensP h, TensP a, const std::string& gn_name, const std::string& conv_name);
  void tape_temb();
  TensP resblock(const std::vector<TensP>& ins, int out_ch, int midx);
  TensP attn(const TensP& x, int midx);
  TensP downsample(const TensP& x, int midx);
  TensP upsample(const TensP& x, int midx);
};

}
```

### meshdiffusion_b200/ops.py

```python
import torch

from . import _native

PRECISIONS = {"bf16": 0, "tf32": 1, "bf16x3": 2}
STAT_WORDS = 4


def stats_to_words(stats):
    v = stats.double()
    hi = torch.round(v / 65536.0)
    lo = torch.round((v - hi * 65536.0) * 16777216.0)
    return torch.stack([lo[..., 0], hi[..., 0], lo[..., 1], hi[..., 1]], dim=-1).to(torch.int64).contiguous()


def words_to_stats(words):
    w = words.double()
    return torch.stack([w[..., 0] / 16777216.0 + w[..., 1] * 65536.0, w[..., 2] / 16777216.0 + w[..., 3] * 65536.0], dim=-1)


def _act_dtype(precision):
    return torch.float32 if precision == "tf32" else torch.bfloat16


def to_ndhwc(x_ncdhw, precision):
    y = x_ncdhw.permute(0, 2, 3, 4, 1).contiguous()
    if precision == "bf16x3":
        hi = y.to(torch.bfloat16)
        lo = (y.float() - hi.float()).to(torch.bfloat16)
        return torch.cat([hi, lo], dim=-1).contiguous()
    return y.to(_act_dtype(precision))


def from_ndhwc(y, precision=None):
    if precision == "bf16x3":
        C = y.shape[-1] // 2
        y = y[..., :C].float() + y[..., C:].float()
    return y.float().permute(0, 4, 1, 2, 3).contiguous()


def conv3d(x, weight, bias=None, stride=1, rowbias=None, residual=None, want_stats=False, precision="bf16"):
    L = _native.lib()
    assert x.is_cuda and x.is_contiguous() and x.dtype == _act_dtype(precision)
    B, Z, Y, X, Cin = x.shape
    parts = 2 if precision == "bf16x3" else 1
    Cin //= parts
    Cout, k = weight.shape[0], weight.shape[2]
    assert weight.shape[1] == Cin
    w = weight.detach().float().contiguous()
    y = torch.empty((B, Z // stride, Y // stride, X // stride, Cout * parts), device=x.device, dtype=x.dtype)
    stats = torch.zeros((B, Cout, STAT_WORDS), device=x.device, dtype=torch.int64) if want_stats else None
    b = bias.detach().float().contiguous() if bias is not None else None
    rb = rowbias.detach().float().contiguous() if rowbias is not None else None
    if residual is not None:
        assert residual.shape == y.shape and residual.dtype == y.dtype and residual.is_contiguous()
    _native.check(L.mdb_conv3d(_native.ptr(x), B, Cin, Z, Y, X, _native.ptr(w), _native.ptr(b), Cout, k, stride,
                               _native.ptr(y), _native.ptr(rb), _native.ptr(residual), _native.ptr(stats),
                               PRECISIONS[precision], _native.current_stream()))
    return (y, words_to_stats(stats)) if want_stats else y


def groupnorm_act(x, stats, gamma, beta, silu=True, precision="bf16"):
    L = _native.lib()
    B, C = x.shape[0], x.shape[-1]
    V = x.numel() // (B * C)
    if precision == "bf16x3":
        C //= 2
    y = torch.empty_like(x)
    stats = stats_to_words(stats)
    g = gamma.detach().float().contiguous()
    bt = beta.detach().float().contiguous()
    _native.check(L.mdb_groupnorm_act(_native.ptr(x), _native.ptr(stats), _native.ptr(g), _native.ptr(bt), _native.ptr(y),
                                      B, V, C, 1 if silu else 0, PRECISIONS[precision], _native.current_stream()))
    return y


def sampler_update(eps, x, noise, mask, beta, std, seed=0, offset=0):
    L = _native.lib()
    B, C = x.shape[0], x.shape[1]
    V = x[0, 0].numel()
    x_mean = torch.empty_like(x)
    _native.check(L.mdb_sampler_update(_native.ptr(eps), _native.ptr(x), _native.ptr(x_mean), _native.ptr(noise),
                                       _native.ptr(mask), float(beta), float(std), V, C, B, seed, offset, None,
                                       _native.current_stream()))
    return x, x_mean


def conv3d_backward(dy, x, weight, stride=1, want_dw=True, want_dx=True, precision="bf16"):
    L = _native.lib()
    if precision not in ("bf16", "bf16x3"):
        raise ValueError("conv3d_backward: precision must be 'bf16' or 'bf16x3'")
    assert dy.dtype == torch.bfloat16 and x.dtype == torch.bfloat16 and dy.is_contiguous() and x.is_contiguous()
    B, Z, Y, X, Cin = x.shape
    parts = 2 if precision == "bf16x3" else 1
    Cin //= parts
    Cout, k = weight.shape[0], weight.shape[2]
    assert weight.shape[1] == Cin and dy.shape[-1] == Cout * parts
    w = weight.detach().float().contiguous()
    dw = torch.zeros_like(w) if want_dw else None
    dx = torch.empty_like(x) if want_dx else None
    _native.check(L.mdb_conv3d_backward_prec(_native.ptr(dy), _native.ptr(x), _native.ptr(w), B, Cin, Cout, Z, Y, X, k, stride,
                                             _native.ptr(dw), _native.ptr(dx), PRECISIONS[precision], _native.current_stream()))
    return dw, dx


def groupnorm_act_backward(x, stats, gamma, beta, da, add=None, silu=True, dropout_p=0.0, seed=0, precision="bf16"):
    L = _native.lib()
    if precision not in ("bf16", "bf16x3"):
        raise ValueError("groupnorm_act_backward: precision must be 'bf16' or 'bf16x3'")
    B, C = x.shape[0], x.shape[-1]
    V = x.numel() // (B * C)
    if precision == "bf16x3":
        C //= 2
    stats = stats_to_words(stats)
    g = gamma.detach().float().contiguous()
    bt = beta.detach().float().contiguous()
    dx = torch.empty_like(x)
    dg = torch.empty(C, device=x.device, dtype=torch.float32)
    db = torch.empty(C, device=x.device, dtype=torch.float32)
    da = da.clone()
    _native.check(L.mdb_groupnorm_act_backward_prec(_native.ptr(x), _native.ptr(stats), _native.ptr(g), _native.ptr(bt),
                                                    _native.ptr(da), _native.ptr(add), _native.ptr(dx), _native.ptr(dg),
                                                    _native.ptr(db), B, V, C, 1 if silu else 0, float(dropout_p), int(seed),
                                                    PRECISIONS[precision], _native.current_stream()))
    return dx, dg, db
```

Baseline: 37.85.

## Add fused flash-attention kernel for UNet attention blocks in inference

```diff
diff --git a/include/meshdiff_b200.h b/include/meshdiff_b200.h
--- a/include/meshdiff_b200.h
+++ b/include/meshdiff_b200.h
@@ -41,6 +41,7 @@
 int mdb_unet_commit(mdb_unet* net, void* stream);
 int mdb_unet_forward(mdb_unet* net, const float* x, const float* labels, float* out, int batch, void* stream);
 int mdb_unet_info(mdb_unet* net, double* flops_per_sample, long long* arena_bytes, int* n_gemm_launches, int* n_steps);
+int mdb_unet_step_name(mdb_unet* net, int i, const char** name);
 int mdb_unet_gemm_ops(mdb_unet* net, int i, const char** name, double* flops, double* fill_bytes);
 int mdb_unet_gemm_slots(mdb_unet* net, int i, int* a_slots, int* b_slots, int* smem_bytes);
 int mdb_unet_gemm_tiles(mdb_unet* net, int i, int* work_items, int* splits, int* ksteps, int* entry_ksteps, int* block_n);
@@ -141,6 +142,8 @@
 int mdb_conv3d(const void* x, int batch, int cin, int z, int y_, int x_, const float* w, const float* bias, int cout,
                int ksize, int stride, void* out, const float* rowbias, const void* residual, long long* stats,
                int precision, void* stream);
+int mdb_attention(const void* q, const void* k, const void* v, void* o, int batch, int V, int C, long long ld, int precision,
+                  int fused, void* stream);
 int mdb_groupnorm_act(const void* x, const long long* stats, const float* gamma, const float* beta, void* y, int batch,
                       long long voxels, int channels, int silu, int precision, void* stream);
 
diff --git a/meshdiffusion_b200/_native.py b/meshdiffusion_b200/_native.py
--- a/meshdiffusion_b200/_native.py
+++ b/meshdiffusion_b200/_native.py
@@ -73,6 +73,7 @@
     "mdb_unet_set_params": (_i, [_vp, _i, _vp, _vp, _vp, _vp]),
     "mdb_unet_forward": (_i, [_vp, _vp, _vp, _vp, _i, _vp]),
     "mdb_unet_info": (_i, [_vp, ctypes.POINTER(_d), ctypes.POINTER(_ll), ctypes.POINTER(_i), ctypes.POINTER(_i)]),
+    "mdb_unet_step_name": (_i, [_vp, _i, ctypes.POINTER(ctypes.c_char_p)]),
     "mdb_unet_gemm_ops": (_i, [_vp, _i, ctypes.POINTER(ctypes.c_char_p), ctypes.POINTER(_d), ctypes.POINTER(_d)]),
     "mdb_unet_gemm_slots": (_i, [_vp, _i, ctypes.POINTER(_i), ctypes.POINTER(_i), ctypes.POINTER(_i)]),
     "mdb_unet_gemm_tiles": (_i, [_vp, _i, ctypes.POINTER(_i), ctypes.POINTER(_i), ctypes.POINTER(_i), ctypes.POINTER(_i),
@@ -108,6 +109,7 @@
     "mdb_allreduce_grads": (_i, [_vp, _vp, _ll, _i, _vp]),
     "mdb_conv3d": (_i, [_vp, _i, _i, _i, _i, _i, _vp, _vp, _i, _i, _i, _vp, _vp, _vp, _vp, _i, _vp]),
     "mdb_groupnorm_act": (_i, [_vp, _vp, _vp, _vp, _vp, _i, _ll, _i, _i, _i, _vp]),
+    "mdb_attention": (_i, [_vp, _vp, _vp, _vp, _i, _i, _i, _ll, _i, _i, _vp]),
     "mdb_conv3d_backward": (_i, [_vp, _vp, _vp, _i, _i, _i, _i, _i, _i, _i, _i, _vp, _vp, _vp]),
     "mdb_groupnorm_act_backward": (_i, [_vp, _vp, _vp, _vp, _vp, _vp, _vp, _vp, _vp, _i, _ll, _i, _i, _f, _u64, _vp]),
     "mdb_conv3d_backward_prec": (_i, [_vp, _vp, _vp, _i, _i, _i, _i, _i, _i, _i, _i, _vp, _vp, _i, _vp]),
diff --git a/meshdiffusion_b200/build.py b/meshdiffusion_b200/build.py
--- a/meshdiffusion_b200/build.py
+++ b/meshdiffusion_b200/build.py
@@ -7,7 +7,7 @@
 CSRC = os.path.join(HERE, "csrc")
 LIBDIR = os.path.join(HERE, "lib")
 LIB = os.path.join(LIBDIR, "libmeshdiff_b200.so")
-SOURCES = ["gemm_host.cu", "wgrad_host.cu", "elementwise.cu", "backward.cu", "unet.cu", "unet_train.cu", "marching_tets.cu", "mesh_ops.cu", "train_ops.cu", "pc_metrics.cu", "emd.cu", "likelihood.cu", "raster.cu", "fit.cu", "depth_partial.cu", "interp.cu", "lfd.cu", "repaint.cu", "api.cu"]
+SOURCES = ["gemm_host.cu", "wgrad_host.cu", "elementwise.cu", "backward.cu", "attention.cu", "unet.cu", "unet_train.cu", "marching_tets.cu", "mesh_ops.cu", "train_ops.cu", "pc_metrics.cu", "emd.cu", "likelihood.cu", "raster.cu", "fit.cu", "depth_partial.cu", "interp.cu", "lfd.cu", "repaint.cu", "api.cu"]
 ARCH_FLAGS = ["-gencode", "arch=compute_90a,code=sm_90a"]
 NVCC_FLAGS = ARCH_FLAGS + [
     "-O3", "-lineinfo", "-std=c++17",
@@ -15,7 +15,7 @@
     "-Xptxas", "-v",
 ]
 SERIALISED_WGMMA = ("C7510", "C7520")
-NO_STACK_KERNELS = ("gemm_tc_kernel", "wgrad_tc_kernel")
+NO_STACK_KERNELS = ("gemm_tc_kernel", "wgrad_tc_kernel", "attention_fused_kernel")
 _PROPS = re.compile(r"Function properties for (\S+)")
 _FRAME = re.compile(r"(\d+) bytes stack frame, (\d+) bytes spill stores, (\d+) bytes spill loads")
 
diff --git a/meshdiffusion_b200/csrc/act_format.cuh b/meshdiffusion_b200/csrc/act_format.cuh
--- a/meshdiffusion_b200/csrc/act_format.cuh
+++ b/meshdiffusion_b200/csrc/act_format.cuh
@@ -102,6 +102,17 @@
   }
 }
 
+template <Precision P>
+__device__ __forceinline__ void store_pair(__nv_bfloat16* hi, long long lo_off, float a, float b) {
+  static_assert(P != kTF32, "store_pair writes bf16 rows");
+  const __nv_bfloat162 h = __floats2bfloat162_rn(a, b);
+  *reinterpret_cast<__nv_bfloat162*>(hi) = h;
+  if constexpr (P == kBF16X3) {
+    const float2 f = __bfloat1622float2(h);
+    *reinterpret_cast<__nv_bfloat162*>(hi + lo_off) = __floats2bfloat162_rn(a - f.x, b - f.y);
+  }
+}
+
 __device__ __forceinline__ unsigned long long drop_hash64(unsigned long long seed, unsigned long long idx) {
   unsigned long long z = idx + seed * 0x9E3779B97F4A7C15ull;
   z = (z ^ (z >> 30)) * 0xBF58476D1CE4E5B9ull;
diff --git a/meshdiffusion_b200/csrc/api.cu b/meshdiffusion_b200/csrc/api.cu
--- a/meshdiffusion_b200/csrc/api.cu
+++ b/meshdiffusion_b200/csrc/api.cu
@@ -1,5 +1,6 @@
 #include "../../include/meshdiff_b200.h"
 #include "unet.h"
+#include "attention.h"
 #include <cstring>
 #include <cmath>
 
@@ -105,6 +106,13 @@
   if (arena) *arena = (long long)n->net->arena_bytes();
   if (ngemm) *ngemm = n->net->num_gemm_launches();
   if (nsteps) *nsteps = n->net->num_steps();
+  MDB_API_END
+}
+
+int mdb_unet_step_name(mdb_unet* n, int i, const char** name) {
+  MDB_API_BEGIN
+  if (i < 0 || i >= n->net->num_steps()) throw std::runtime_error("mdb: step index out of range");
+  *name = n->net->step_name(i).c_str();
   MDB_API_END
 }
 
@@ -426,6 +434,55 @@
   g.repack(s);
   g.launch(s);
   MDB_CUDA_CHECK(cudaStreamSynchronize(s));
+  MDB_API_END
+}
+
+int mdb_attention(const void* q, const void* k, const void* v, void* o, int B, int V, int C, long long ld, int precision,
+                  int fused, void* stream) {
+  MDB_API_BEGIN
+  cudaStream_t s = (cudaStream_t)stream;
+  const Precision pr = precision_from_int(precision);
+  const float alpha = 1.0f / std::sqrt((float)C);
+  if (fused) {
+    launch_attention(make_attention_params(q, k, v, ld, o, C, B, V, C, alpha, pr), B, s);
+    MDB_CUDA_CHECK(cudaStreamSynchronize(s));
+    return 0;
+  }
+  const int es = esize(pr);
+  void* vT = nullptr; float* S = nullptr;
+  MDB_CUDA_CHECK(cudaMalloc(&vT, (size_t)B * C * V * es * parts(pr)));
+  MDB_CUDA_CHECK(cudaMalloc((void**)&S, (size_t)B * V * V * 4));
+  try {
+    if (pr == kBF16X3) {
+      launch_transpose_vc(v, 2 * ld, 0, vT, B, V, C, es, s, 2 * V);
+      launch_transpose_vc(v, 2 * ld, ld, (__nv_bfloat16*)vT + V, B, V, C, es, s, 2 * V);
+    } else {
+      launch_transpose_vc(v, ld, 0, vT, B, V, C, es, s);
+    }
+    GemmOp gqk;
+    gqk.set_output_strided(pr, V, 1, 1, B, V, S, V, 0, 0, (long long)V * V, true);
+    Act qa; qa.ptr = const_cast<void*>(q); qa.C = C; qa.ld = ld; qa.X = V; qa.Y = 1; qa.Z = 1; qa.B = B;
+    gqk.add_pointwise_w({qa}, nullptr);
+    gqk.set_b_activation(const_cast<void*>(k), C, V, B, ld, (long long)V * ld);
+    gqk.set_alpha(alpha);
+    gqk.finalize();
+    gqk.upload(s);
+    gqk.launch(s);
+    launch_softmax_rows(S, (long long)B * V, V, pr, s);
+    GemmOp gpv;
+    gpv.set_output_strided(pr, V, 1, 1, B, C, o, C, 0, 0, (long long)V * C, false);
+    Act pa; pa.ptr = S; pa.C = V; pa.ld = (pr == kBF16) ? 2 * V : V; pa.X = V; pa.Y = 1; pa.Z = 1; pa.B = B;
+    gpv.add_pointwise_w({pa}, nullptr);
+    gpv.set_b_activation(vT, V, C, B, V, (long long)C * V);
+    gpv.finalize();
+    gpv.upload(s);
+    gpv.launch(s);
+    MDB_CUDA_CHECK(cudaStreamSynchronize(s));
+  } catch (...) {
+    cudaFree(vT); cudaFree(S);
+    throw;
+  }
+  cudaFree(vT); cudaFree(S);
   MDB_API_END
 }
 
diff --git a/meshdiffusion_b200/csrc/attention.cu b/meshdiffusion_b200/csrc/attention.cu
--- /dev/null
+++ b/meshdiffusion_b200/csrc/attention.cu
@@ -0,0 +1,251 @@
+#include "attention.h"
+#include "gemm_host.h"
+#include "ptx.cuh"
+
+namespace mdb {
+
+constexpr int kAttnThreads = 384;
+constexpr int kAttnBoxRowBytes = 128;
+constexpr int kAttnQBox = kAttnBlockQ * kAttnBoxRowBytes;
+constexpr int kAttnTileBytes = 32768;
+constexpr int kAttnRegsProducer = 40, kAttnRegsConsumer = 232;
+
+template <Precision P>
+struct AttnCfg {
+  static constexpr int kParts = parts(P);
+  static constexpr int kBc = P == kBF16X3 ? 32 : 64;
+  static constexpr int kBox = kBc * kAttnBoxRowBytes;
+  static_assert(kParts * (kAttnC / 64) * kBox == kAttnTileBytes, "a K / V tile fills one slot");
+  static constexpr int kQBytes = kParts * (kAttnC / 64) * kAttnQBox;
+  static constexpr int kBarBytes = 256;
+  static constexpr int kSlots = (kMaxDynSmem - 1024 - kBarBytes - kQBytes) / kAttnTileBytes;
+  static_assert(kSlots >= 2, "two ring slots at least");
+  static constexpr int kSmem = 1024 + kQBytes + kSlots * kAttnTileBytes + kBarBytes;
+};
+
+template <Precision P>
+__global__ void __launch_bounds__(kAttnThreads, 1) attention_fused_kernel(const __grid_constant__ AttnParams p) {
+  using Cfg = AttnCfg<P>;
+  constexpr int kParts = Cfg::kParts, kBc = Cfg::kBc, kBox = Cfg::kBox, NS = Cfg::kSlots;
+  constexpr int kCB = kAttnC / 64;
+  extern __shared__ uint8_t smem_raw[];
+  uint8_t* smem = reinterpret_cast<uint8_t*>((reinterpret_cast<uintptr_t>(smem_raw) + 1023) & ~uintptr_t(1023));
+  const uint32_t q_s = smem_u32(smem), ring = q_s + Cfg::kQBytes;
+  const uint32_t q_full = ring + NS * kAttnTileBytes, full = q_full + 8, empty = full + 8 * NS;
+
+  const int warp = __shfl_sync(0xffffffffu, (int)(threadIdx.x >> 5), 0), lane = threadIdx.x & 31;
+  const int q0 = (int)blockIdx.x * kAttnBlockQ, b = (int)blockIdx.y;
+  const int n_tiles = p.V / kBc;
+  const int ld = (int)p.ld;
+
+  if (warp == 0 && lane == 0) {
+    tma_prefetch_desc(&p.qmap);
+    tma_prefetch_desc(&p.kmap);
+    tma_prefetch_desc(&p.vmap);
+  }
+  if (warp == 1 && lane == 0) {
+    mbar_init(q_full, 1);
+    for (int i = 0; i < NS; ++i) { mbar_init(full + 8 * i, 1); mbar_init(empty + 8 * i, 2); }
+    fence_barrier_init();
+    fence_proxy_async();
+  }
+  __syncthreads();
+
+  if (warp < 4) {
+    setmaxnreg_dec<kAttnRegsProducer>();
+    if (warp == 0) {
+      if (elect_one()) {
+        mbar_expect_tx(q_full, Cfg::kQBytes);
+        for (int part = 0; part < kParts; ++part)
+          for (int cb = 0; cb < kCB; ++cb)
+            tma_load_3d(&p.qmap, q_full, q_s + (part * kCB + cb) * kAttnQBox, part * ld + cb * 64, q0, b);
+      }
+      __syncwarp();
+      uint32_t s = 0, ph = 0;
+      for (int j = 0; j < 2 * n_tiles; ++j) {
+        mbar_wait(empty + 8 * s, ph ^ 1);
+        if (elect_one()) {
+          const CUtensorMap* map = (j & 1) ? &p.vmap : &p.kmap;
+          const uint32_t base = ring + s * kAttnTileBytes, bar = full + 8 * s;
+          mbar_expect_tx(bar, kAttnTileBytes);
+          for (int part = 0; part < kParts; ++part)
+            for (int cb = 0; cb < kCB; ++cb)
+              tma_load_3d(map, bar, base + (part * kCB + cb) * kBox, part * ld + cb * 64, (j >> 1) * kBc, b);
+        }
+        __syncwarp();
+        if (++s == (uint32_t)NS) { s = 0; ph ^= 1; }
+      }
+    }
+  } else {
+    setmaxnreg_inc<kAttnRegsConsumer>();
+    const int wg = (warp - 4) >> 2, wt = threadIdx.x & 127;
+    const uint32_t q_rows = q_s + wg * 64 * kAttnBoxRowBytes;
+    float o[kAttnC / 2];
+#pragma unroll
+    for (int i = 0; i < kAttnC / 2; ++i) o[i] = 0.f;
+    float m0 = -INFINITY, m1 = -INFINITY, l0 = 0.f, l1 = 0.f;
+    uint32_t s = 0, ph = 0;
+    mbar_wait(q_full, 0);
+#pragma unroll 1
+    for (int j = 0; j < n_tiles; ++j) {
+      float sc[kBc / 2];
+      mbar_wait(full + 8 * s, ph);
+      {
+        const uint32_t kb = ring + s * kAttnTileBytes;
+        wgmma_fence();
+        if constexpr (P == kBF16X3) {
+#pragma unroll
+          for (int cb = 0; cb < kCB; ++cb)
+#pragma unroll
+            for (int k = 0; k < 4; ++k) {
+              wgmma_kmajor<kBc, false>(sc, kdesc(q_rows + cb * kAttnQBox) + 2 * k, kdesc(kb + (kCB + cb) * kBox) + 2 * k, (cb | k) ? 1u : 0u);
+              wgmma_kmajor<kBc, false>(sc, kdesc(q_rows + (kCB + cb) * kAttnQBox) + 2 * k, kdesc(kb + cb * kBox) + 2 * k, 1u);
+            }
+        }
+#pragma unroll
+        for (int cb = 0; cb < kCB; ++cb)
+#pragma unroll
+          for (int k = 0; k < 4; ++k)
+            wgmma_kmajor<kBc, false>(sc, kdesc(q_rows + cb * kAttnQBox) + 2 * k, kdesc(kb + cb * kBox) + 2 * k, (P == kBF16X3 || cb | k) ? 1u : 0u);
+        wgmma_commit();
+        wgmma_wait<0>();
+        fence_operands(sc);
+        if (wt == 0) mbar_arrive(empty + 8 * s);
+        if (++s == (uint32_t)NS) { s = 0; ph ^= 1; }
+      }
+      float mx0 = m0, mx1 = m1;
+#pragma unroll
+      for (int i = 0; i < kBc / 8; ++i) {
+        sc[4 * i] *= p.scale_log2; sc[4 * i + 1] *= p.scale_log2;
+        sc[4 * i + 2] *= p.scale_log2; sc[4 * i + 3] *= p.scale_log2;
+        mx0 = fmaxf(mx0, fmaxf(sc[4 * i], sc[4 * i + 1]));
+        mx1 = fmaxf(mx1, fmaxf(sc[4 * i + 2], sc[4 * i + 3]));
+      }
+      mx0 = fmaxf(mx0, __shfl_xor_sync(0xffffffffu, mx0, 1));
+      mx0 = fmaxf(mx0, __shfl_xor_sync(0xffffffffu, mx0, 2));
+      mx1 = fmaxf(mx1, __shfl_xor_sync(0xffffffffu, mx1, 1));
+      mx1 = fmaxf(mx1, __shfl_xor_sync(0xffffffffu, mx1, 2));
+      float c0, c1;
+      asm("ex2.approx.ftz.f32 %0, %1;" : "=f"(c0) : "f"(m0 - mx0));
+      asm("ex2.approx.ftz.f32 %0, %1;" : "=f"(c1) : "f"(m1 - mx1));
+      m0 = mx0; m1 = mx1;
+      l0 *= c0; l1 *= c1;
+#pragma unroll
+      for (int i = 0; i < kBc / 8; ++i) {
+#pragma unroll
+        for (int e = 0; e < 4; ++e) {
+          float pe;
+          asm("ex2.approx.ftz.f32 %0, %1;" : "=f"(pe) : "f"(sc[4 * i + e] - (e < 2 ? mx0 : mx1)));
+          sc[4 * i + e] = pe;
+          if (e < 2) l0 += pe; else l1 += pe;
+        }
+      }
+#pragma unroll
+      for (int i = 0; i < kAttnC / 8; ++i) {
+        o[4 * i] *= c0; o[4 * i + 1] *= c0;
+        o[4 * i + 2] *= c1; o[4 * i + 3] *= c1;
+      }
+      uint32_t ph_[kBc / 16][4], pl_[kBc / 16][4];
+#pragma unroll
+      for (int k = 0; k < kBc / 16; ++k)
+#pragma unroll
+        for (int r = 0; r < 4; ++r) {
+          const float a = sc[8 * k + 2 * r], c = sc[8 * k + 2 * r + 1];
+          const __nv_bfloat162 h = __floats2bfloat162_rn(a, c);
+          ph_[k][r] = *reinterpret_cast<const uint32_t*>(&h);
+          if constexpr (P == kBF16X3) {
+            const float2 f = __bfloat1622float2(h);
+            const __nv_bfloat162 lo = __floats2bfloat162_rn(a - f.x, c - f.y);
+            pl_[k][r] = *reinterpret_cast<const uint32_t*>(&lo);
+          }
+        }
+      mbar_wait(full + 8 * s, ph);
+      {
+        const uint32_t vb = ring + s * kAttnTileBytes;
+        wgmma_fence();
+#pragma unroll
+        for (int k = 0; k < kBc / 16; ++k) {
+          const uint64_t vh = make_wgmma_desc(vb + k * 16 * kAttnBoxRowBytes, kBox, 1024);
+          if constexpr (P == kBF16X3) {
+            const uint64_t vl = make_wgmma_desc(vb + kCB * kBox + k * 16 * kAttnBoxRowBytes, kBox, 1024);
+            wgmma_m64n256k16_bf16_rs<1>(o, pl_[k], vh, 1u);
+            wgmma_m64n256k16_bf16_rs<1>(o, ph_[k], vl, 1u);
+          }
+          wgmma_m64n256k16_bf16_rs<1>(o, ph_[k], vh, 1u);
+        }
+        wgmma_commit();
+        wgmma_wait<0>();
+        fence_operands(o);
+        if (wt == 0) mbar_arrive(empty + 8 * s);
+        if (++s == (uint32_t)NS) { s = 0; ph ^= 1; }
+      }
+    }
+    l0 += __shfl_xor_sync(0xffffffffu, l0, 1);
+    l0 += __shfl_xor_sync(0xffffffffu, l0, 2);
+    l1 += __shfl_xor_sync(0xffffffffu, l1, 1);
+    l1 += __shfl_xor_sync(0xffffffffu, l1, 2);
+    const float inv0 = 1.f / l0, inv1 = 1.f / l1;
+    const int g = 16 * (warp & 3) + (lane >> 2), t = lane & 3;
+    const long long pitch = (long long)kParts * p.ldo;
+    __nv_bfloat16* r0 = reinterpret_cast<__nv_bfloat16*>(p.out) + ((long long)b * p.V + q0 + 64 * wg + g) * pitch + 2 * t;
+    __nv_bfloat16* r1 = r0 + 8 * pitch;
+#pragma unroll
+    for (int i = 0; i < kAttnC / 8; ++i) {
+      store_pair<P>(r0 + 8 * i, p.ldo, o[4 * i] * inv0, o[4 * i + 1] * inv0);
+      store_pair<P>(r1 + 8 * i, p.ldo, o[4 * i + 2] * inv1, o[4 * i + 3] * inv1);
+    }
+  }
+}
+
+static MapDesc attn_map(const void* base, long long ld, int max_batch, int V, int C, Precision prec, int box_rows) {
+  const int np = parts(prec);
+  MapDesc d;
+  d.base = const_cast<void*>(base);
+  d.rank = 3;
+  d.dims[0] = (uint64_t)((np - 1) * ld + C);
+  d.dims[1] = (uint64_t)V;
+  d.dims[2] = (uint64_t)max_batch;
+  d.strides[0] = (uint64_t)(np * ld * 2);
+  d.strides[1] = (uint64_t)V * np * ld * 2;
+  d.box[0] = 64; d.box[1] = (uint32_t)box_rows; d.box[2] = 1;
+  return d;
+}
+
+AttnParams make_attention_params(const void* q, const void* k, const void* v, long long ld, void* out, long long ldo,
+                                 int max_batch, int V, int C, float alpha, Precision prec) {
+  if (!attention_fused_ok(prec, C, V)) throw std::runtime_error("mdb: the fused attention kernel takes bf16 / split-bf16 rows of 256 channels over a multiple of 128 positions");
+  if (ld < C || ldo < C || (ld * 2) % 16 || (ldo * 2) % 16) throw std::runtime_error("mdb: attention row pitches must hold C channels and be multiples of 8");
+  for (const void* ptr : {q, k, v, (const void*)out})
+    if (reinterpret_cast<uintptr_t>(ptr) % 16) throw std::runtime_error("mdb: attention operands must be 16-byte aligned");
+  AttnParams p{};
+  const int bc = prec == kBF16X3 ? AttnCfg<kBF16X3>::kBc : AttnCfg<kBF16>::kBc;
+  encode_map(&p.qmap, prec, attn_map(q, ld, max_batch, V, C, prec, kAttnBlockQ));
+  encode_map(&p.kmap, prec, attn_map(k, ld, max_batch, V, C, prec, bc));
+  encode_map(&p.vmap, prec, attn_map(v, ld, max_batch, V, C, prec, bc));
+  p.out = out; p.ldo = ldo; p.ld = ld; p.V = V; p.max_batch = max_batch;
+  p.scale_log2 = alpha * 1.4426950408889634f;
+  p.prec = prec;
+  return p;
+}
+
+template <Precision P>
+static void launch_impl(const AttnParams& p, int B, cudaStream_t s) {
+  static bool configured[64] = {};
+  auto kern = attention_fused_kernel<P>;
+  int dev = 0;
+  MDB_CUDA_CHECK(cudaGetDevice(&dev));
+  if (dev >= 64 || !configured[dev]) {
+    MDB_CUDA_CHECK(cudaFuncSetAttribute(kern, cudaFuncAttributeMaxDynamicSharedMemorySize, AttnCfg<P>::kSmem));
+    if (dev < 64) configured[dev] = true;
+  }
+  kern<<<dim3(p.V / kAttnBlockQ, B), kAttnThreads, AttnCfg<P>::kSmem, s>>>(p);
+  MDB_CUDA_CHECK(cudaGetLastError());
+}
+
+void launch_attention(const AttnParams& p, int B, cudaStream_t s) {
+  if (B < 1 || B > p.max_batch) throw std::runtime_error("mdb: attention batch out of range");
+  if (p.prec == kBF16X3) launch_impl<kBF16X3>(p, B, s);
+  else launch_impl<kBF16>(p, B, s);
+}
+
+}
diff --git a/meshdiffusion_b200/csrc/attention.h b/meshdiffusion_b200/csrc/attention.h
--- /dev/null
+++ b/meshdiffusion_b200/csrc/attention.h
@@ -0,0 +1,31 @@
+#pragma once
+#include <cuda.h>
+#include <cuda_runtime.h>
+#include "act_format.cuh"
+
+namespace mdb {
+
+constexpr int kAttnC = 256;
+constexpr int kAttnBlockQ = 128;
+constexpr int kAttnMinCtas = 64;
+
+struct AttnParams {
+  CUtensorMap qmap, kmap, vmap;
+  void* out;
+  long long ldo;
+  long long ld;
+  int V;
+  int max_batch;
+  float scale_log2;
+  Precision prec;
+};
+
+inline bool attention_fused_ok(Precision prec, int C, long long V) {
+  return prec != kTF32 && C == kAttnC && V % kAttnBlockQ == 0;
+}
+
+AttnParams make_attention_params(const void* q, const void* k, const void* v, long long ld, void* out, long long ldo,
+                                 int max_batch, int V, int C, float alpha, Precision prec);
+void launch_attention(const AttnParams& p, int B, cudaStream_t s);
+
+}
diff --git a/meshdiffusion_b200/csrc/ptx.cuh b/meshdiffusion_b200/csrc/ptx.cuh
--- a/meshdiffusion_b200/csrc/ptx.cuh
+++ b/meshdiffusion_b200/csrc/ptx.cuh
@@ -150,6 +150,17 @@
       "%128, %129, p, 1, 1, %131, %132;\n\t}"
       : "+f"(d[0]), "+f"(d[1]), "+f"(d[2]), "+f"(d[3]), "+f"(d[4]), "+f"(d[5]), "+f"(d[6]), "+f"(d[7]), "+f"(d[8]), "+f"(d[9]), "+f"(d[10]), "+f"(d[11]), "+f"(d[12]), "+f"(d[13]), "+f"(d[14]), "+f"(d[15]), "+f"(d[16]), "+f"(d[17]), "+f"(d[18]), "+f"(d[19]), "+f"(d[20]), "+f"(d[21]), "+f"(d[22]), "+f"(d[23]), "+f"(d[24]), "+f"(d[25]), "+f"(d[26]), "+f"(d[27]), "+f"(d[28]), "+f"(d[29]), "+f"(d[30]), "+f"(d[31]), "+f"(d[32]), "+f"(d[33]), "+f"(d[34]), "+f"(d[35]), "+f"(d[36]), "+f"(d[37]), "+f"(d[38]), "+f"(d[39]), "+f"(d[40]), "+f"(d[41]), "+f"(d[42]), "+f"(d[43]), "+f"(d[44]), "+f"(d[45]), "+f"(d[46]), "+f"(d[47]), "+f"(d[48]), "+f"(d[49]), "+f"(d[50]), "+f"(d[51]), "+f"(d[52]), "+f"(d[53]), "+f"(d[54]), "+f"(d[55]), "+f"(d[56]), "+f"(d[57]), "+f"(d[58]), "+f"(d[59]), "+f"(d[60]), "+f"(d[61]), "+f"(d[62]), "+f"(d[63]), "+f"(d[64]), "+f"(d[65]), "+f"(d[66]), "+f"(d[67]), "+f"(d[68]), "+f"(d[69]), "+f"(d[70]), "+f"(d[71]), "+f"(d[72]), "+f"(d[73]), "+f"(d[74]), "+f"(d[75]), "+f"(d[76]), "+f"(d[77]), "+f"(d[78]), "+f"(d[79]), "+f"(d[80]), "+f"(d[81]), "+f"(d[82]), "+f"(d[83]), "+f"(d[84]), "+f"(d[85]), "+f"(d[86]), "+f"(d[87]), "+f"(d[88]), "+f"(d[89]), "+f"(d[90]), "+f"(d[91]), "+f"(d[92]), "+f"(d[93]), "+f"(d[94]), "+f"(d[95]), "+f"(d[96]), "+f"(d[97]), "+f"(d[98]), "+f"(d[99]), "+f"(d[100]), "+f"(d[101]), "+f"(d[102]), "+f"(d[103]), "+f"(d[104]), "+f"(d[105]), "+f"(d[106]), "+f"(d[107]), "+f"(d[108]), "+f"(d[109]), "+f"(d[110]), "+f"(d[111]), "+f"(d[112]), "+f"(d[113]), "+f"(d[114]), "+f"(d[115]), "+f"(d[116]), "+f"(d[117]), "+f"(d[118]), "+f"(d[119]), "+f"(d[120]), "+f"(d[121]), "+f"(d[122]), "+f"(d[123]), "+f"(d[124]), "+f"(d[125]), "+f"(d[126]), "+f"(d[127])
       : "l"(a), "l"(b), "r"(scale_d), "n"(TA), "n"(TB));
+}
+
+template <int TB>
+__device__ __forceinline__ void wgmma_m64n256k16_bf16_rs(float (&d)[128], const uint32_t (&a)[4], uint64_t b, uint32_t scale_d) {
+  asm volatile(
+      "{\n\t.reg .pred p;\n\tsetp.ne.b32 p, %133, 0;\n\t"
+      "wgmma.mma_async.sync.aligned.m64n256k16.f32.bf16.bf16 "
+      "{%0, %1, %2, %3, %4, %5, %6, %7, %8, %9, %10, %11, %12, %13, %14, %15, %16, %17, %18, %19, %20, %21, %22, %23, %24, %25, %26, %27, %28, %29, %30, %31, %32, %33, %34, %35, %36, %37, %38, %39, %40, %41, %42, %43, %44, %45, %46, %47, %48, %49, %50, %51, %52, %53, %54, %55, %56, %57, %58, %59, %60, %61, %62, %63, %64, %65, %66, %67, %68, %69, %70, %71, %72, %73, %74, %75, %76, %77, %78, %79, %80, %81, %82, %83, %84, %85, %86, %87, %88, %89, %90, %91, %92, %93, %94, %95, %96, %97, %98, %99, %100, %101, %102, %103, %104, %105, %106, %107, %108, %109, %110, %111, %112, %113, %114, %115, %116, %117, %118, %119, %120, %121, %122, %123, %124, %125, %126, %127}, "
+      "{%128, %129, %130, %131}, %132, p, 1, 1, %134;\n\t}"
+      : "+f"(d[0]), "+f"(d[1]), "+f"(d[2]), "+f"(d[3]), "+f"(d[4]), "+f"(d[5]), "+f"(d[6]), "+f"(d[7]), "+f"(d[8]), "+f"(d[9]), "+f"(d[10]), "+f"(d[11]), "+f"(d[12]), "+f"(d[13]), "+f"(d[14]), "+f"(d[15]), "+f"(d[16]), "+f"(d[17]), "+f"(d[18]), "+f"(d[19]), "+f"(d[20]), "+f"(d[21]), "+f"(d[22]), "+f"(d[23]), "+f"(d[24]), "+f"(d[25]), "+f"(d[26]), "+f"(d[27]), "+f"(d[28]), "+f"(d[29]), "+f"(d[30]), "+f"(d[31]), "+f"(d[32]), "+f"(d[33]), "+f"(d[34]), "+f"(d[35]), "+f"(d[36]), "+f"(d[37]), "+f"(d[38]), "+f"(d[39]), "+f"(d[40]), "+f"(d[41]), "+f"(d[42]), "+f"(d[43]), "+f"(d[44]), "+f"(d[45]), "+f"(d[46]), "+f"(d[47]), "+f"(d[48]), "+f"(d[49]), "+f"(d[50]), "+f"(d[51]), "+f"(d[52]), "+f"(d[53]), "+f"(d[54]), "+f"(d[55]), "+f"(d[56]), "+f"(d[57]), "+f"(d[58]), "+f"(d[59]), "+f"(d[60]), "+f"(d[61]), "+f"(d[62]), "+f"(d[63]), "+f"(d[64]), "+f"(d[65]), "+f"(d[66]), "+f"(d[67]), "+f"(d[68]), "+f"(d[69]), "+f"(d[70]), "+f"(d[71]), "+f"(d[72]), "+f"(d[73]), "+f"(d[74]), "+f"(d[75]), "+f"(d[76]), "+f"(d[77]), "+f"(d[78]), "+f"(d[79]), "+f"(d[80]), "+f"(d[81]), "+f"(d[82]), "+f"(d[83]), "+f"(d[84]), "+f"(d[85]), "+f"(d[86]), "+f"(d[87]), "+f"(d[88]), "+f"(d[89]), "+f"(d[90]), "+f"(d[91]), "+f"(d[92]), "+f"(d[93]), "+f"(d[94]), "+f"(d[95]), "+f"(d[96]), "+f"(d[97]), "+f"(d[98]), "+f"(d[99]), "+f"(d[100]), "+f"(d[101]), "+f"(d[102]), "+f"(d[103]), "+f"(d[104]), "+f"(d[105]), "+f"(d[106]), "+f"(d[107]), "+f"(d[108]), "+f"(d[109]), "+f"(d[110]), "+f"(d[111]), "+f"(d[112]), "+f"(d[113]), "+f"(d[114]), "+f"(d[115]), "+f"(d[116]), "+f"(d[117]), "+f"(d[118]), "+f"(d[119]), "+f"(d[120]), "+f"(d[121]), "+f"(d[122]), "+f"(d[123]), "+f"(d[124]), "+f"(d[125]), "+f"(d[126]), "+f"(d[127])
+      : "r"(a[0]), "r"(a[1]), "r"(a[2]), "r"(a[3]), "l"(b), "r"(scale_d), "n"(TB));
 }
 
 template <int N, bool TF32>
diff --git a/meshdiffusion_b200/csrc/unet.cu b/meshdiffusion_b200/csrc/unet.cu
--- a/meshdiffusion_b200/csrc/unet.cu
+++ b/meshdiffusion_b200/csrc/unet.cu
@@ -1,4 +1,5 @@
 #include "unet.h"
+#include "attention.h"
 #include <algorithm>
 #include <cmath>
 
@@ -245,40 +246,56 @@
     gemm_step(steps_, g);
   }
   release(hn);
-  TensP vT = new_act(C, R, false);
-  {
-    const void* src = qkv->ptr; void* dst = vT->ptr;
-    if (prec_ == kBF16X3) {
-      add_step("attn" + std::to_string(midx) + ".vT", [=](cudaStream_t s, int B) {
-        launch_transpose_vc(src, 6 * C, 2 * C, dst, B, V, C, es, s, 2 * V);
-        launch_transpose_vc(src, 6 * C, 5 * C, (__nv_bfloat16*)dst + V, B, V, C, es, s, 2 * V);
-      });
-    } else
-    add_step("attn" + std::to_string(midx) + ".vT", [=](cudaStream_t s, int B) { launch_transpose_vc(src, 3 * C, 2 * C, dst, B, V, C, es, s); });
-  }
-  auto S = std::make_shared<Tens>();
-  S->bytes = (size_t)mb * V * V * 4;
-  S->off = arena_.alloc(S->bytes);
-  S->ptr = at(S->off);
-  TensP O = new_act(C, R, false);
-  GemmOp* gqk = new_gemm("attn" + std::to_string(midx) + ".qk");
-  gqk->set_output_strided(prec_, V, 1, 1, mb, V, S->ptr, V, 0, 0, (long long)V * V, true);
-  Act q; q.ptr = qkv->ptr; q.C = C; q.ld = 3 * C; q.X = V; q.Y = 1; q.Z = 1; q.B = mb;
-  gqk->add_pointwise_w({q}, nullptr);
-  gqk->set_b_activation((char*)qkv->ptr + (size_t)C * es, C, V, mb, 3 * C, (long long)V * 3 * C);
-  gqk->set_alpha(1.0f / std::sqrt((float)C));
-  gemm_step(steps_, gqk);
-  float* sp = (float*)S->ptr; const Precision pr = prec_;
-  add_step("attn" + std::to_string(midx) + ".softmax", [=](cudaStream_t s, int B) { launch_softmax_rows(sp, (long long)B * V, V, pr, s); });
-  GemmOp* gpv = new_gemm("attn" + std::to_string(midx) + ".pv");
-  gpv->set_output_strided(prec_, V, 1, 1, mb, C, O->ptr, C, 0, 0, (long long)V * C, false);
-  Act pa; pa.ptr = S->ptr; pa.C = V; pa.ld = (prec_ == kBF16) ? 2 * V : V; pa.X = V; pa.Y = 1; pa.Z = 1; pa.B = mb;
-  gpv->add_pointwise_w({pa}, nullptr);
-  gpv->set_b_activation(vT->ptr, V, C, mb, V, (long long)C * V);
-  gemm_step(steps_, gpv);
-  if (!train_) arena_.release(S->off);
-  { arena_.release(vT->off); vT->live = false; }
-  release(qkv);
+  const std::string an = "attn" + std::to_string(midx);
+  const float alpha = 1.0f / std::sqrt((float)C);
+  std::shared_ptr<Tens> S;
+  TensP O;
+  if (!train_ && attention_fused_ok(prec_, C, V) && (long long)mb * (V / kAttnBlockQ) >= kAttnMinCtas) {
+    O = new_act(C, R, false);
+    auto ap = std::make_shared<AttnParams>();
+    if (!dry_) {
+      char* base = (char*)qkv->ptr;
+      *ap = make_attention_params(base, base + (size_t)C * es, base + (size_t)2 * C * es, 3 * C, O->ptr, C, mb, V, C, alpha, prec_);
+    }
+    add_step(an + ".flash.pv", [ap](cudaStream_t s, int B) { launch_attention(*ap, B, s); });
+    fused_flops_ += 4.0 * mb * (double)V * V * C;
+    release(qkv);
+  } else {
+    TensP vT = new_act(C, R, false);
+    {
+      const void* src = qkv->ptr; void* dst = vT->ptr;
+      if (prec_ == kBF16X3) {
+        add_step("attn" + std::to_string(midx) + ".vT", [=](cudaStream_t s, int B) {
+          launch_transpose_vc(src, 6 * C, 2 * C, dst, B, V, C, es, s, 2 * V);
+          launch_transpose_vc(src, 6 * C, 5 * C, (__nv_bfloat16*)dst + V, B, V, C, es, s, 2 * V);
+        });
+      } else
+      add_step("attn" + std::to_string(midx) + ".vT", [=](cudaStream_t s, int B) { launch_transpose_vc(src, 3 * C, 2 * C, dst, B, V, C, es, s); });
+    }
+    S = std::make_shared<Tens>();
+    S->bytes = (size_t)mb * V * V * 4;
+    S->off = arena_.alloc(S->bytes);
+    S->ptr = at(S->off);
+    O = new_act(C, R, false);
+    GemmOp* gqk = new_gemm("attn" + std::to_string(midx) + ".qk");
+    gqk->set_output_strided(prec_, V, 1, 1, mb, V, S->ptr, V, 0, 0, (long long)V * V, true);
+    Act q; q.ptr = qkv->ptr; q.C = C; q.ld = 3 * C; q.X = V; q.Y = 1; q.Z = 1; q.B = mb;
+    gqk->add_pointwise_w({q}, nullptr);
+    gqk->set_b_activation((char*)qkv->ptr + (size_t)C * es, C, V, mb, 3 * C, (long long)V * 3 * C);
+    gqk->set_alpha(alpha);
+    gemm_step(steps_, gqk);
+    float* sp = (float*)S->ptr; const Precision pr = prec_;
+    add_step("attn" + std::to_string(midx) + ".softmax", [=](cudaStream_t s, int B) { launch_softmax_rows(sp, (long long)B * V, V, pr, s); });
+    GemmOp* gpv = new_gemm("attn" + std::to_string(midx) + ".pv");
+    gpv->set_output_strided(prec_, V, 1, 1, mb, C, O->ptr, C, 0, 0, (long long)V * C, false);
+    Act pa; pa.ptr = S->ptr; pa.C = V; pa.ld = (prec_ == kBF16) ? 2 * V : V; pa.X = V; pa.Y = 1; pa.Z = 1; pa.B = mb;
+    gpv->add_pointwise_w({pa}, nullptr);
+    gpv->set_b_activation(vT->ptr, V, C, mb, V, (long long)C * V);
+    gemm_step(steps_, gpv);
+    if (!train_) arena_.release(S->off);
+    { arena_.release(vT->off); vT->live = false; }
+    release(qkv);
+  }
   TensP out = new_act(C, R, true);
   GemmOp* g3 = new_gemm("attn" + std::to_string(midx) + ".nin3");
   g3->set_output(prec_, R, R, R, mb, C, out->ptr, C, false);
@@ -363,6 +380,7 @@
   arena_.reset();
   stats_cursor_ = 0;
   dense_cursor_ = 0;
+  fused_flops_ = 0;
   steps_.clear(); commit_steps_.clear(); bwd_steps_.clear();
   gemms_.clear(); commit_gemms_.clear(); bwd_gemms_.clear(); wgrads_.clear();
   grad_ready_.clear();
@@ -520,7 +538,7 @@
     tape_.clear();
     if (arena_.in_use() != 0) throw std::runtime_error("mdb: training plan leaked " + std::to_string(arena_.in_use()) + " arena bytes");
   }
-  flops_ = 0;
+  flops_ = fused_flops_;
   for (auto& g : gemms_) flops_ += g->flops;
   bwd_flops_ = 0;
   for (auto& g : bwd_gemms_) bwd_flops_ += g->flops;
diff --git a/meshdiffusion_b200/csrc/unet.h b/meshdiffusion_b200/csrc/unet.h
--- a/meshdiffusion_b200/csrc/unet.h
+++ b/meshdiffusion_b200/csrc/unet.h
@@ -96,6 +96,7 @@
   int num_gemm_launches() const { return (int)gemms_.size(); }
   const GemmOp& gemm(int i) const { return *gemms_.at(i); }
   int num_steps() const { return (int)steps_.size(); }
+  const std::string& step_name(int i) const { return steps_.at(i).name; }
   const UNetConfig& cfg() const { return cfg_; }
   std::vector<std::pair<std::string, float>> profile(const float* x, const float* labels, float* out, int B, cudaStream_t s);
 
@@ -118,6 +119,7 @@
   std::vector<Step> steps_, commit_steps_;
   bool committed_ = false;
   double flops_ = 0;
+  double fused_flops_ = 0;
   struct FwdGraph { const float* x; const float* labels; float* out; int B; int uses; cudaGraphExec_t exec; };
   std::vector<FwdGraph> graphs_;
   cudaStream_t capture_stream_ = nullptr;
diff --git a/meshdiffusion_b200/ops.py b/meshdiffusion_b200/ops.py
--- a/meshdiffusion_b200/ops.py
+++ b/meshdiffusion_b200/ops.py
@@ -57,6 +57,21 @@
                                _native.ptr(y), _native.ptr(rb), _native.ptr(residual), _native.ptr(stats),
                                PRECISIONS[precision], _native.current_stream()))
     return (y, words_to_stats(stats)) if want_stats else y
+
+
+def attention(qkv, precision="bf16", fused=True):
+    L = _native.lib()
+    assert qkv.is_cuda and qkv.is_contiguous() and qkv.dtype == _act_dtype(precision)
+    B, V, W = qkv.shape
+    parts = 2 if precision == "bf16x3" else 1
+    C = W // (3 * parts)
+    assert W == 3 * C * parts
+    o = torch.empty((B, V, C * parts), device=qkv.device, dtype=qkv.dtype)
+    es = qkv.element_size()
+    base = qkv.data_ptr()
+    _native.check(L.mdb_attention(base, base + C * es, base + 2 * C * es, _native.ptr(o), B, V, C, 3 * C,
+                                  PRECISIONS[precision], 1 if fused else 0, _native.current_stream()))
+    return o
 
 
 def groupnorm_act(x, stats, gamma, beta, silu=True, precision="bf16"):
```

Result: faster. 38.50 (median of 6 runs) (+1.7%).
